# MengAiDev/SmokePhysAI

Hardware: AMD Instinct MI355X
Metric: simulated+encoded frames/sec at 256^2 grid, batch 64 (higher is better)
Workload: dtype f32 stencil + bf16x3 encoder (split-bf16 MFMA, fp32 accumulate)

## Files before the change

### smokephysai_amd/csrc/encoder.hip

```cpp
#include "encoder.h"

#include <stdlib.h>

#include "encoder_tile.h"

namespace smk {

typedef float f32x16 __attribute__((ext_vector_type(16)));

constexpr int ENC_TH = 8, ENC_TW = 32;
constexpr int ENC_AH = ENC_TH + 2, ENC_AW = ENC_TW + 2;
constexpr int ENC_XH = ENC_TH + 8, ENC_XW = ENC_TW + 8;
constexpr int ENC_ACS = ENC_AH * ENC_AW;

__global__ void k_fold_weights(smk_encoder_weights w, EncoderDev e) {
    int t = blockIdx.x * blockDim.x + threadIdx.x;
    if (t < 64) {
        float s = w.bn1_w[t] / sqrtf(w.bn1_var[t] + 1e-5f);
        e.s1[t] = s;
        e.t1[t] = (w.conv1_b[t] - w.bn1_mean[t]) * s + w.bn1_b[t];
    }
    if (t < 128) {
        float s = w.bn2_w[t] / sqrtf(w.bn2_var[t] + 1e-5f);
        e.s2[t] = s;
        e.t2[t] = (w.conv2_b[t] - w.bn2_mean[t]) * s + w.bn2_b[t];
    }
    if (t < 64 * 49) e.w1[t] = w.conv1_w[t];
    if (t < 9 * 64 * 128) {
        int o = t % 128, c = (t / 128) % 64, tap = t / (128 * 64);
        e.w2t[t] = w.conv2_w[((size_t)o * 64 + c) * 9 + tap];
    }
    __bf16 *w1p = reinterpret_cast<__bf16 *>(e.w1p), *w2q = reinterpret_cast<__bf16 *>(e.w2q);
    if (t < 64 * 64) {
        int c = t / 64, k = t % 64, ki = k >> 3, kj = k & 7;
        float v = (ki < 7 && kj < 7) ? w.conv1_w[c * 49 + ki * 7 + kj] : 0.f;
        __bf16 hi = (__bf16)v;
        w1p[t] = hi;
        w1p[64 * 64 + t] = (__bf16)(v - (float)hi);
    }
    if (t < 36 * 128 * 16) {
        int cc = t % 16, o = (t / 16) % 128, ks = t / (16 * 128);
        int tap = ks >> 2, c = (ks & 3) * 16 + cc;
        float v = w.conv2_w[((size_t)o * 64 + c) * 9 + tap];
        __bf16 hi = (__bf16)v;
        w2q[((size_t)(ks * 2 + 0) * 128 + o) * 16 + cc] = hi;
        w2q[((size_t)(ks * 2 + 1) * 128 + o) * 16 + cc] = (__bf16)(v - (float)hi);
        __bf16 *w2s = reinterpret_cast<__bf16 *>(e.w2s);
        const int ks2 = tap * 2 + (c >> 5), c32 = c & 31;
        w2s[((size_t)(ks2 * 2 + 0) * 128 + o) * 32 + c32] = hi;
        w2s[((size_t)(ks2 * 2 + 1) * 128 + o) * 32 + c32] = (__bf16)(v - (float)hi);
    }
}

__global__ __launch_bounds__(256) void k_quant_w2(smk_encoder_weights w, EncoderDev e) {
    __shared__ float red[256];
    __shared__ int sh_h, sh_l;
    const int o = blockIdx.x, tid = threadIdx.x;
    if (tid == 0) { sh_h = 0; sh_l = 0; }
    float m = 0.f;
    for (int k = tid; k < 576; k += 256) m = fmaxf(m, fabsf(w.conv2_w[(size_t)o * 576 + k]));
    red[tid] = m;
    __syncthreads();
    for (int sft = 128; sft > 0; sft >>= 1) {
        if (tid < sft) red[tid] = fmaxf(red[tid], red[tid + sft]);
        __syncthreads();
    }
    const float wmax = red[0];
    const float sw = wmax > 0.f ? wmax / 32512.0f : 1.0f;
    if (tid == 0) e.sw2[o] = sw;
    int sum_h = 0, sum_l = 0;
    for (int k = tid; k < 576; k += 256) {
        const int c = k / 9, tap = k - 9 * c;
        const int q = (int)rintf(w.conv2_w[(size_t)o * 576 + k] / sw);
        const int h = (q + 128) >> 8, l = q - (h << 8);
        const int ks = tap * 2 + (c >> 5), cc = c & 31;
        e.w2i[((size_t)(ks * 2 + 0) * 128 + o) * 32 + cc] = (signed char)h;
        e.w2i[((size_t)(ks * 2 + 1) * 128 + o) * 32 + cc] = (signed char)l;
        sum_h += h; sum_l += l;
    }
    atomicAdd(&sh_h, sum_h);
    atomicAdd(&sh_l, sum_l);
    __syncthreads();
    if (tid == 0) { e.wsum[o] = 128 * sh_h; e.wsum[128 + o] = 128 * sh_l; }
}

hipError_t launch_fold_weights(const smk_encoder_weights &w, const EncoderDev &e, hipStream_t st) {
    hipLaunchKernelGGL(k_quant_w2, dim3(128), dim3(256), 0, st, w, e);
    int n = 9 * 64 * 128;
    hipLaunchKernelGGL(k_fold_weights, dim3((n + 255) / 256), dim3(256), 0, st, w, e);
    return hipGetLastError();
}

template <int NC>
__device__ __forceinline__ void conv1_pixel(const float (&patch)[49], const float *__restrict__ w1,
                                            const float *__restrict__ s1, const float *__restrict__ t1, int c0,
                                            float (&out)[NC]) {
#pragma unroll
    for (int cc = 0; cc < NC; ++cc) {
        const float *wc = w1 + (c0 + cc) * 49;
        float acc = 0.f;
#pragma unroll
        for (int t = 0; t < 49; ++t) acc = fmaf(patch[t], wc[t], acc);
        float y = fmaf(acc, s1[c0 + cc], t1[c0 + cc]);
        out[cc] = y > 0.f ? y : 0.f;
    }
}

__global__ __launch_bounds__(256) void k_conv1_only(const float *frames, int64_t fstride, int H, int W, EncoderDev e, float *act) {
    int b = blockIdx.z;
    int j = blockIdx.x * 64 + threadIdx.x, i = blockIdx.y * 4 + threadIdx.y;
    if (i >= H || j >= W) return;
    const float *x = frames + (size_t)b * fstride;
    float patch[49];
#pragma unroll
    for (int ki = 0; ki < 7; ++ki)
#pragma unroll
        for (int kj = 0; kj < 7; ++kj) {
            int ii = i + ki - 3, jj = j + kj - 3;
            patch[ki * 7 + kj] = (ii >= 0 && ii < H && jj >= 0 && jj < W) ? x[(size_t)ii * W + jj] : 0.f;
        }
#pragma unroll 1
    for (int c0 = 0; c0 < 64; c0 += 4) {
        float o[4];
        conv1_pixel<4>(patch, e.w1, e.s1, e.t1, c0, o);
#pragma unroll
        for (int cc = 0; cc < 4; ++cc) act[(((size_t)b * 64 + c0 + cc) * H + i) * W + j] = o[cc];
    }
}

hipError_t launch_conv1_only(const float *frames, int64_t fstride, int B, int H, int W, const EncoderDev &e, float *act,
                             hipStream_t st) {
    dim3 grid(cdiv(W, 64), cdiv(H, 4), B), block(64, 4);
    hipLaunchKernelGGL(k_conv1_only, grid, block, 0, st, frames, fstride, H, W, e, act);
    return hipGetLastError();
}

constexpr int POOL_THREADS = 256;

template <int V>
__global__ __launch_bounds__(POOL_THREADS) void k_encoder_pool_partials_tokens(const float *__restrict__ partials, float *__restrict__ features,
                                                                               int ncells, int lg_tr, int lg_tc, float inv) {
    typedef float vec_t __attribute__((ext_vector_type(V)));
    constexpr int PER = 128 / V;
    const int idx = blockIdx.x * POOL_THREADS + threadIdx.x, cell = idx / PER, o = (idx - cell * PER) * V;
    if (cell >= ncells) return;
    const int b = cell >> 10, pi = (cell >> 5) & 31, pj = cell & 31, tiles_x = 32 << lg_tc;
    const float *p = partials + (((size_t)b * (32 << lg_tr) + ((size_t)pi << lg_tr)) * tiles_x + (pj << lg_tc)) * 128 + o;
    vec_t sum = *reinterpret_cast<const vec_t *>(p);
    for (int tr = 0; tr < (1 << lg_tr); ++tr)
        for (int tc = (tr == 0); tc < (1 << lg_tc); ++tc) sum += *reinterpret_cast<const vec_t *>(p + ((size_t)tr * tiles_x + tc) * 128);
    *reinterpret_cast<vec_t *>(features + (size_t)cell * 128 + o) = sum * inv;
}

__global__ __launch_bounds__(POOL_THREADS) void k_encoder_pool_partials(const float *__restrict__ partials, float *__restrict__ features,
                                                                        int lg_tr, int lg_tc, float inv) {
    __shared__ float cells[32][129];
    const int tid = threadIdx.x, b = blockIdx.x >> 5, pi = blockIdx.x & 31, tiles_x = 32 << lg_tc;
    const float *row = partials + ((size_t)b * (32 << lg_tr) + ((size_t)pi << lg_tr)) * tiles_x * 128;
    for (int i = tid; i < 32 * 32; i += POOL_THREADS) {
        const int pj = i >> 5, o = (i & 31) * 4;
        const float *p = row + (size_t)(pj << lg_tc) * 128 + o;
        float4 sum = *reinterpret_cast<const float4 *>(p);
        for (int tr = 0; tr < (1 << lg_tr); ++tr)
            for (int tc = (tr == 0); tc < (1 << lg_tc); ++tc) {
                const float4 v = *reinterpret_cast<const float4 *>(p + ((size_t)tr * tiles_x + tc) * 128);
                sum.x += v.x; sum.y += v.y; sum.z += v.z; sum.w += v.w;
            }
        cells[pj][o] = sum.x * inv; cells[pj][o + 1] = sum.y * inv; cells[pj][o + 2] = sum.z * inv; cells[pj][o + 3] = sum.w * inv;
    }
    __syncthreads();
    for (int i = tid; i < 128 * 32; i += POOL_THREADS) {
        const int o = i >> 5, pj = i & 31;
        features[((size_t)b * 128 + o) * 1024 + pi * 32 + pj] = cells[pj][o];
    }
}

static hipError_t launch_pool_partials(const float *partials, float *features, int B, int H, bool tokens, hipStream_t st) {
    const int PS = H / 32, lg_tr = PS == 16 ? 1 : 2, lg_tc = lg_tr - 1;
    const float inv = 1.0f / (float)(PS * PS);
    if (!tokens) {
        hipLaunchKernelGGL(k_encoder_pool_partials, dim3(B * 32), dim3(POOL_THREADS), 0, st, partials, features, lg_tr, lg_tc, inv);
    } else if ((reinterpret_cast<uintptr_t>(features) & 15) == 0) {
        hipLaunchKernelGGL(k_encoder_pool_partials_tokens<4>, dim3(B * 1024 * 32 / POOL_THREADS), dim3(POOL_THREADS), 0, st, partials,
                           features, B * 1024, lg_tr, lg_tc, inv);
    } else {
        hipLaunchKernelGGL(k_encoder_pool_partials_tokens<1>, dim3(B * 1024 * 128 / POOL_THREADS), dim3(POOL_THREADS), 0, st, partials,
                           features, B * 1024, lg_tr, lg_tc, inv);
    }
    return hipGetLastError();
}

void EncoderPartials::release() {
    if (buf) (void)hipFree(buf);
    for (void *p : retired) (void)hipFree(p);
    retired.clear();
    buf = nullptr;
    floats = 0;
}

hipError_t EncoderPartials::acquire(int B, int H, int W, hipStream_t st, float **out) {
    *out = nullptr;
    if (H / 32 < 16) return hipSuccess;
    const size_t need = (size_t)B * (H / B3_TH) * (W / B3_TW) * 128;
    std::lock_guard<std::mutex> lk(mu);
    if (floats < need) {
        hipStreamCaptureStatus cs = hipStreamCaptureStatusNone;
        if (hipStreamIsCapturing(st, &cs) != hipSuccess) (void)hipGetLastError();
        if (cs != hipStreamCaptureStatusNone) return hipErrorStreamCaptureUnsupported;
        float *p = nullptr;
        const hipError_t err = hipMalloc((void **)&p, need * sizeof(float));
        if (err != hipSuccess) return err;
        if (buf) retired.push_back(buf);
        buf = p;
        floats = need;
    }
    *out = buf;
    return hipSuccess;
}

constexpr int LDS_XS = ENC_XH * ENC_XW;
constexpr int LDS_A1 = 64 * ENC_ACS;
constexpr int LDS_W2 = 64 * 128;
constexpr int LDS_F32_TOTAL = LDS_XS + LDS_A1 + 2 * LDS_W2;
constexpr int A2_PITCH = 129;

template <int PS>
__global__ __launch_bounds__(512) void k_encoder_f32(const float *__restrict__ frames, int64_t fstride, int H, int W,
                                                     EncoderDev e, float *__restrict__ features) {
    extern __shared__ __attribute__((aligned(16))) float lds[];
    float *xs = lds, *a1s = lds + LDS_XS, *w2s = lds + LDS_XS + LDS_A1;
    const int tid = threadIdx.x, lane = tid & 63;
    const int wave = __builtin_amdgcn_readfirstlane(tid >> 6);
    const int b = blockIdx.z, r0 = blockIdx.y * ENC_TH, c0 = blockIdx.x * ENC_TW;
    const float *x = frames + (size_t)b * fstride;

    for (int k = tid; k < LDS_XS; k += 512) {
        int ii = r0 - 4 + k / ENC_XW, jj = c0 - 4 + k % ENC_XW;
        xs[k] = (ii >= 0 && ii < H && jj >= 0 && jj < W) ? x[(size_t)ii * W + jj] : 0.f;
    }
    float4 wreg[4];
    {
        const float4 *src = reinterpret_cast<const float4 *>(e.w2t);
#pragma unroll
        for (int q = 0; q < 4; ++q) wreg[q] = src[q * 512 + tid];
    }
    __syncthreads();

    for (int task = wave; task < 48; task += 8) {
        const int chunk = task % 6, cq = task / 6;
        const int pix = chunk * 64 + lane;
        if (pix < ENC_ACS) {
            const int ar = pix / ENC_AW, ac = pix % ENC_AW;
            const int ii = r0 - 1 + ar, jj = c0 - 1 + ac;
            float o[8];
            if (ii >= 0 && ii < H && jj >= 0 && jj < W) {
                float patch[49];
#pragma unroll
                for (int ki = 0; ki < 7; ++ki)
#pragma unroll
                    for (int kj = 0; kj < 7; ++kj) patch[ki * 7 + kj] = xs[(ar + ki) * ENC_XW + ac + kj];
                conv1_pixel<8>(patch, e.w1, e.s1, e.t1, cq * 8, o);
            } else {
#pragma unroll
                for (int cc = 0; cc < 8; ++cc) o[cc] = 0.f;
            }
#pragma unroll
            for (int cc = 0; cc < 8; ++cc) a1s[(cq * 8 + cc) * ENC_ACS + pix] = o[cc];
        }
    }
    {
        float4 *dst = reinterpret_cast<float4 *>(w2s);
#pragma unroll
        for (int q = 0; q < 4; ++q) dst[q * 512 + tid] = wreg[q];
    }
    __syncthreads();

    f32x16 acc[4];
#pragma unroll
    for (int n = 0; n < 4; ++n)
#pragma unroll
        for (int r = 0; r < 16; ++r) acc[n][r] = 0.f;
    const int l31 = lane & 31, hi = lane >> 5;
    for (int tap = 0; tap < 9; ++tap) {
        if (tap + 1 < 9) {
            const float4 *src = reinterpret_cast<const float4 *>(e.w2t + (size_t)(tap + 1) * LDS_W2);
#pragma unroll
            for (int q = 0; q < 4; ++q) wreg[q] = src[q * 512 + tid];
        }
        const int ki = tap / 3, kj = tap % 3;
        const float *ap = a1s + hi * ENC_ACS + (wave + ki) * ENC_AW + l31 + kj;
        const float *bp = w2s + (tap & 1) * LDS_W2 + hi * 128 + l31;
#pragma unroll 4
        for (int cp = 0; cp < 32; ++cp) {
            float a = ap[cp * 2 * ENC_ACS];
#pragma unroll
            for (int n = 0; n < 4; ++n) {
                float bv = bp[cp * 2 * 128 + n * 32];
                acc[n] = __builtin_amdgcn_mfma_f32_32x32x2f32(a, bv, acc[n], 0, 0, 0);
            }
        }
        if (tap + 1 < 9) {
            float4 *dst = reinterpret_cast<float4 *>(w2s + ((tap + 1) & 1) * LDS_W2);
#pragma unroll
            for (int q = 0; q < 4; ++q) dst[q * 512 + tid] = wreg[q];
        }
        __syncthreads();
    }

    float *a2s = lds;
#pragma unroll
    for (int n = 0; n < 4; ++n) {
        const int o = n * 32 + l31;
        const float s = e.s2[o], t = e.t2[o];
#pragma unroll
        for (int r = 0; r < 16; ++r) {
            const int col = (r & 3) + 8 * (r >> 2) + 4 * hi;
            float y = fmaf(acc[n][r], s, t);
            a2s[(wave * ENC_TW + col) * A2_PITCH + o] = y > 0.f ? y : 0.f;
        }
    }
    __syncthreads();
    if constexpr (PS >= 16) {
        if (tid < 256) {
            const int o = tid & 127, half = tid >> 7;
            float sum = 0.f;
            for (int rr = 0; rr < ENC_TH; ++rr)
                for (int q = 0; q < B3_TW; ++q) sum += a2s[(rr * ENC_TW + half * B3_TW + q) * A2_PITCH + o];
            const size_t tile = ((size_t)b * (H / B3_TH) + blockIdx.y) * (W / B3_TW) + 2 * blockIdx.x + half;
            features[tile * 128 + o] = sum;
        }
    } else {
        constexpr int CELLS_R = ENC_TH / PS, CELLS_C = ENC_TW / PS;
        const int OW = 32, OHW = 32 * 32;
        for (int k = tid; k < CELLS_R * CELLS_C * 128; k += 512) {
            const int o = k & 127, cell = k >> 7, cr = cell / CELLS_C, cc = cell % CELLS_C;
            float sum = 0.f;
            for (int rr = 0; rr < PS; ++rr)
                for (int q = 0; q < PS; ++q) sum += a2s[((cr * PS + rr) * ENC_TW + cc * PS + q) * A2_PITCH + o];
            const int pi = r0 / PS + cr, pj = c0 / PS + cc;
            features[((size_t)b * 128 + o) * OHW + pi * OW + pj] = sum * (1.0f / (PS * PS));
        }
    }
}

hipError_t launch_encoder_f32(const float *frames, int64_t fstride, int B, int H, int W, const EncoderDev &e,
                              float *features, hipStream_t st, float *partials) {
    const int PS = H / 32;
    if (PS >= 16 && !partials) return hipErrorInvalidValue;
    dim3 grid(W / ENC_TW, H / ENC_TH, B), block(512);
    size_t lds_bytes = sizeof(float) * (size_t)(LDS_F32_TOTAL > 256 * A2_PITCH ? LDS_F32_TOTAL : 256 * A2_PITCH);
    once_per_device((const void *)k_encoder_f32<8>, [&] {
        (void)hipFuncSetAttribute((const void *)k_encoder_f32<2>, hipFuncAttributeMaxDynamicSharedMemorySize, (int)lds_bytes);
        (void)hipFuncSetAttribute((const void *)k_encoder_f32<4>, hipFuncAttributeMaxDynamicSharedMemorySize, (int)lds_bytes);
        (void)hipFuncSetAttribute((const void *)k_encoder_f32<8>, hipFuncAttributeMaxDynamicSharedMemorySize, (int)lds_bytes);
        (void)hipFuncSetAttribute((const void *)k_encoder_f32<16>, hipFuncAttributeMaxDynamicSharedMemorySize, (int)lds_bytes);
    });
    switch (PS) {
        case 2: hipLaunchKernelGGL(k_encoder_f32<2>, grid, block, lds_bytes, st, frames, fstride, H, W, e, features); break;
        case 4: hipLaunchKernelGGL(k_encoder_f32<4>, grid, block, lds_bytes, st, frames, fstride, H, W, e, features); break;
        case 8: hipLaunchKernelGGL(k_encoder_f32<8>, grid, block, lds_bytes, st, frames, fstride, H, W, e, features); break;
        case 16:
        case 32: {
            hipLaunchKernelGGL(k_encoder_f32<16>, grid, block, lds_bytes, st, frames, fstride, H, W, e, partials);
            const hipError_t err = hipGetLastError();
            return err != hipSuccess ? err : launch_pool_partials(partials, features, B, H, false, st);
        }
        default: return hipErrorInvalidValue;
    }
    return hipGetLastError();
}

typedef __bf16 bf16x4 __attribute__((ext_vector_type(4)));

constexpr int B3_XH = B3_TH + 9, B3_XW = B3_TW + 9;
constexpr int B3_XS_BYTES = ((B3_XH * B3_XW * 4 + 15) / 16) * 16;
constexpr int B3_A1_PITCH = 144;
constexpr int B3_A1_ROW = B3_AW * B3_A1_PITCH + 32;
constexpr int B3_A1_BYTES = (B3_TH + 2) * B3_A1_ROW;
template <bool X3> constexpr int b3_lds_bytes() { return B3_XS_BYTES + (X3 ? 2 : 1) * B3_A1_BYTES; }

template <bool X3>
__device__ __forceinline__ void mma3(f32x16 &acc, const bf16x8 &ah, const bf16x8 &al, const bf16x8 &bh, const bf16x8 &bl) {
    if (X3) {
        acc = __builtin_amdgcn_mfma_f32_32x32x16_bf16(al, bh, acc, 0, 0, 0);
        acc = __builtin_amdgcn_mfma_f32_32x32x16_bf16(ah, bl, acc, 0, 0, 0);
    }
    acc = __builtin_amdgcn_mfma_f32_32x32x16_bf16(ah, bh, acc, 0, 0, 0);
}

__device__ __forceinline__ float bn_relu(float a, float s, float t) {
    float y = fmaf(a, s, t);
    return y > 0.f ? y : 0.f;
}

constexpr int B3_W1_PITCH = 144;
constexpr int B3_W1_BYTES = 64 * B3_W1_PITCH;
constexpr int B3_ST_BYTES = 2 * 64 * 4;
template <bool X3> constexpr int b3_lds_total() { return b3_lds_bytes<X3>() + (X3 ? 2 : 1) * B3_W1_BYTES + B3_ST_BYTES; }

struct SkipArgs {
    const unsigned long long *masks = nullptr;
    int *count = nullptr;
    const float *table = nullptr;
    int nbands = 0, lg_band_tiles = 0, bands_per_frame = 0;
};
constexpr int scan_rows_for(int tiles_x) { return tiles_x <= 16 ? 4 : 64 / tiles_x; }
constexpr int ENC_FRAME_FEATS = 128 * 1024;
constexpr int SKIP_CHUNKS = 256, SKIP_SLATE = 16;
struct SkipLds {
    int cpre[SKIP_CHUNKS + 1];
    int wsum[4];
    int slate[SKIP_SLATE];
};

__device__ __forceinline__ int skip_lookup(const SkipLds &s, const SkipArgs &sa, int k) {
    int c = 0;
#pragma unroll
    for (int step = SKIP_CHUNKS / 2; step >= 1; step >>= 1)
        if (s.cpre[c + step] <= k) c += step;
    int n = k - s.cpre[c];
    int j = c * ((sa.nbands + SKIP_CHUNKS - 1) / SKIP_CHUNKS);
    unsigned long long m = sa.masks[j];
    for (int pc = __popcll(m); n >= pc; pc = __popcll(m)) {
        n -= pc;
        m = sa.masks[++j];
    }
    int pos = 0;
#pragma unroll
    for (int w = 32; w >= 1; w >>= 1) {
        const int cnt = __popcll((m >> pos) & ((1ull << w) - 1));
        if (n >= cnt) {
            n -= cnt;
            pos += w;
        }
    }
    return (j << sa.lg_band_tiles) + pos;
}

__device__ __forceinline__ void skip_slate(SkipLds &s, const SkipArgs &sa, int r0, int nrun) {
    const int i = threadIdx.x;
    if (i < SKIP_SLATE) {
        const long long k = (long long)blockIdx.x + (long long)(r0 + i) * gridDim.x;
        if (k < nrun) s.slate[i] = skip_lookup(s, sa, (int)k);
    }
}

__device__ __forceinline__ int tiles_to_run(SkipLds &s, const SkipArgs &sa, int ntiles) {
    if (!sa.masks) return ntiles;
    const int tid = threadIdx.x, lane = tid & 63, wave = tid >> 6;
    const int cs = (sa.nbands + SKIP_CHUNKS - 1) / SKIP_CHUNKS;
    int c = 0;
    for (int j = tid * cs, je = min(j + cs, sa.nbands); j < je; ++j) c += __popcll(sa.masks[j]);
    int inc = c;
#pragma unroll
    for (int d = 1; d < 64; d <<= 1) {
        const int v = __shfl_up(inc, d);
        if (lane >= d) inc += v;
    }
    if (lane == 63) s.wsum[wave] = inc;
    __syncthreads();
    int base = 0;
    for (int w = 0; w < wave; ++w) base += s.wsum[w];
    s.cpre[tid] = base + inc - c;
    if (tid == SKIP_CHUNKS - 1) s.cpre[SKIP_CHUNKS] = base + inc;
    __syncthreads();
    const int nrun = __builtin_amdgcn_readfirstlane(s.cpre[SKIP_CHUNKS]);
    if (blockIdx.x == 0 && tid == 0) *sa.count = nrun;
    if (nrun != ntiles) {
        skip_slate(s, sa, 0, nrun);
        __syncthreads();
    }
    return nrun;
}
__device__ __forceinline__ int tile_at(SkipLds &s, const SkipArgs &sa, bool listed, int round, int k, int nrun) {
    if (!listed) return k;
    if (round > 0 && (round & (SKIP_SLATE - 1)) == 0) {
        skip_slate(s, sa, round, nrun);
        __syncthreads();
    }
    return __builtin_amdgcn_readfirstlane(s.slate[round & (SKIP_SLATE - 1)]);
}

template <int PS, bool TOKENS>
__device__ __forceinline__ void skip_fill(const SkipArgs &sa, int lg_tiles_x, float *__restrict__ features) {
    constexpr bool PART = PS >= 16;
    constexpr int CR = PART ? 1 : B3_TH / PS, CC = PART ? 1 : B3_TW / PS;
    constexpr int VW = TOKENS || PART ? 4 : (CC < 4 ? CC : 4), VPR = TOKENS || PART ? 1 : CC / VW, ROWV = CC * 32;
    constexpr int UPT = TOKENS || PART ? CR * ROWV : 128 * CR * VPR;
    constexpr int UNR = 4;
    typedef float vec_t __attribute__((ext_vector_type(VW)));
    const int tid = threadIdx.x, tiles_x = 1 << lg_tiles_x, band_tiles = 1 << sa.lg_band_tiles, total = band_tiles * UPT;
    const unsigned long long full = band_tiles == 64 ? ~0ull : (1ull << band_tiles) - 1;
    for (int band = blockIdx.x; band < sa.nbands; band += gridDim.x) {
        const unsigned long long mv = sa.masks[band];
        const unsigned long long m = ((unsigned long long)__builtin_amdgcn_readfirstlane((unsigned int)(mv >> 32)) << 32) |
                                     (unsigned int)__builtin_amdgcn_readfirstlane((unsigned int)mv);
        if (m == full) continue;
        const int lg_rows = PART ? sa.lg_band_tiles - lg_tiles_x : 2;
        const int b = band / sa.bands_per_frame, ty0 = (band - b * sa.bands_per_frame) << lg_rows;
        float *out = features + (size_t)b * (PART ? (size_t)sa.bands_per_frame << (sa.lg_band_tiles + 7) : (size_t)ENC_FRAME_FEATS);
        for (int i0 = tid; i0 < total; i0 += 256 * UNR) {
            vec_t v[UNR];
            int off[UNR];
#pragma unroll
            for (int j = 0; j < UNR; ++j) {
                const int i = i0 + 256 * j, tl = i / UPT, u = i - tl * UPT;
                off[j] = -1;
                if (i >= total || ((m >> tl) & 1)) continue;
                const int ty = ty0 + (tl >> lg_tiles_x), tx = tl & (tiles_x - 1);
                if (PART) {
                    off[j] = ((ty << lg_tiles_x) + tx) * 128 + u * 4;
                } else if (TOKENS) {
                    const int a = u / ROWV, q = u - a * ROWV;
                    off[j] = ((ty * CR + a) * 32 + tx * CC) * 128 + q * 4;
                } else {
                    const int vv = u % VPR, a = (u / VPR) % CR, o = u / (VPR * CR);
                    off[j] = o * 1024 + (ty * CR + a) * 32 + tx * CC + vv * VW;
                }
                v[j] = *reinterpret_cast<const vec_t *>(sa.table + off[j]);
            }
#pragma unroll
            for (int j = 0; j < UNR; ++j)
                if (off[j] >= 0) __builtin_nontemporal_store(v[j], reinterpret_cast<vec_t *>(out + off[j]));
        }
    }
}
__device__ __forceinline__ bool skip_fill_first() { return (blockIdx.x / 256) & 1; }


template <int PARTS>
__device__ __forceinline__ void conv1_stage(const EncoderDev &e, unsigned char *w1s, float *st1) {
    const int tid = threadIdx.x;
    if (tid < 128) st1[tid] = tid < 64 ? e.s1[tid] : e.t1[tid - 64];
    const uint4 *src = reinterpret_cast<const uint4 *>(e.w1p);
    for (int c = tid; c < PARTS * 64 * 8; c += 256) {
        const int row = c >> 3, u = c & 7;
        *reinterpret_cast<uint4 *>(w1s + row * B3_W1_PITCH + u * 16) = src[c];
    }
}

struct TileSrc {
    const float *frames;
    int64_t fstride;
    int H, W, lg_tiles_x, lg_tiles_per_frame;
    __device__ __forceinline__ void decode(int t, int &b, int &r0, int &c0) const {
        b = t >> lg_tiles_per_frame;
        const int rem = t & ((1 << lg_tiles_per_frame) - 1);
        r0 = (rem >> lg_tiles_x) * B3_TH;
        c0 = (rem & ((1 << lg_tiles_x) - 1)) * B3_TW;
    }
    __device__ __forceinline__ float fetch(int t, int k) const {
        if (k >= B3_XH * B3_XW) return 0.f;
        int bb, rr0, cc0;
        decode(t, bb, rr0, cc0);
        const int row = k / B3_XW, col = k - row * B3_XW;
        const int ii = rr0 - 4 + row, jj = cc0 - 4 + col;
        const bool ok = row < B3_XH - 1 && col < B3_XW - 1 && ii >= 0 && ii < H && jj >= 0 && jj < W;
        return ok ? frames[(size_t)bb * fstride + (size_t)ii * W + jj] : 0.f;
    }
};

template <class T, class Word>
__device__ __forceinline__ void halo_to_lds(T *xs, float v0, float v1, Word word) {
    const int tid = threadIdx.x;
    xs[tid] = word(v0);
    if (tid + 256 < B3_XH * B3_XW) xs[tid + 256] = word(v1);
}

struct TileWalk {
    int k, nrun, round, t, tn;
    bool listed;

    template <int PS, bool TOKENS, class T, class Word>
    __device__ __forceinline__ void begin(SkipLds &skl, const SkipArgs &sa, const TileSrc &src, int ntiles, int stagger,
                                          float *__restrict__ features, T *xs, Word word) {
        k = blockIdx.x;
        nrun = tiles_to_run(skl, sa, ntiles);
        listed = nrun != ntiles;
        round = 0;
        t = k < nrun ? tile_at(skl, sa, listed, 0, k, nrun) : 0;
        if (listed && skip_fill_first()) skip_fill<PS, TOKENS>(sa, src.lg_tiles_x, features);
        else if (stagger > 0 && ((blockIdx.x / 256) & 1))
            for (int i = 0; i < stagger; ++i) __builtin_amdgcn_s_sleep(127);
        const int tid = threadIdx.x;
        if (k < nrun) halo_to_lds(xs, src.fetch(t, tid), src.fetch(t, tid + 256), word);
        __syncthreads();
    }
    __device__ __forceinline__ void next(SkipLds &skl, const SkipArgs &sa, const TileSrc &src, float &xr0, float &xr1) {
        const int kn = k + gridDim.x;
        ++round;
        tn = kn < nrun ? tile_at(skl, sa, listed, round, kn, nrun) : 0;
        xr0 = 0.f;
        xr1 = 0.f;
        if (kn < nrun) {
            const int tid = threadIdx.x;
            xr0 = src.fetch(tn, tid);
            xr1 = src.fetch(tn, tid + 256);
        }
    }
    template <int PS, bool TOKENS>
    __device__ __forceinline__ void end(const SkipArgs &sa, const TileSrc &src, float *__restrict__ features) const {
        if (listed && !skip_fill_first()) {
            __builtin_amdgcn_s_setprio(0);
            skip_fill<PS, TOKENS>(sa, src.lg_tiles_x, features);
        }
    }
};

template <int A1_ROW, int A1_PITCH>
__device__ __forceinline__ void x_frags(const float *xs, int pb, int r0, int c0, int H, int W, bf16x8 (&xh)[4], bf16x8 (&xl)[4],
                                        int &aoff, bool &valid, bool &inimg) {
    const int r = threadIdx.x & 31, hi = (threadIdx.x >> 5) & 1;
    const int pix = pb * 32 + r;
    valid = pix < B3_APIX;
    const int pc = valid ? pix : B3_APIX - 1;
    const int ar = pc / B3_AW, ac = pc - ar * B3_AW;
    const int ii = r0 - 1 + ar, jj = c0 - 1 + ac;
    inimg = valid && ii >= 0 && ii < H && jj >= 0 && jj < W;
    aoff = ar * A1_ROW + ac * A1_PITCH;
    const float *xp = xs + (ar + hi) * B3_XW + ac;
#pragma unroll
    for (int s = 0; s < 4; ++s)
#pragma unroll
        for (int j = 0; j < 8; ++j) {
            __bf16 vh, vl;
            split_bf16(xp[s * 2 * B3_XW + j], vh, vl);
            xh[s][j] = vh; xl[s][j] = vl;
        }
}

template <bool X3>
__device__ __forceinline__ void conv1_both(const unsigned char *w1s, const bf16x8 (&xh)[4], const bf16x8 (&xl)[4], f32x16 &acc0,
                                           f32x16 &acc1) {
    const int r = threadIdx.x & 31, hi = (threadIdx.x >> 5) & 1;
#pragma unroll
    for (int g = 0; g < 16; ++g) { acc0[g] = 0.f; acc1[g] = 0.f; }
    const unsigned char *wrow = w1s + r * B3_W1_PITCH + 8 * hi * 2;
#pragma unroll
    for (int s = 0; s < 4; ++s) {
        const bf16x8 a0h = *reinterpret_cast<const bf16x8 *>(wrow + s * 32);
        const bf16x8 a1hh = *reinterpret_cast<const bf16x8 *>(wrow + 32 * B3_W1_PITCH + s * 32);
        const bf16x8 a0l = X3 ? *reinterpret_cast<const bf16x8 *>(wrow + B3_W1_BYTES + s * 32) : a0h;
        const bf16x8 a1l_ = X3 ? *reinterpret_cast<const bf16x8 *>(wrow + B3_W1_BYTES + 32 * B3_W1_PITCH + s * 32) : a1hh;
        mma3<X3>(acc0, a0h, a0l, xh[s], xl[s]);
        mma3<X3>(acc1, a1hh, a1l_, xh[s], xl[s]);
    }
}
template <bool X3>
__device__ __forceinline__ void conv1_one(const unsigned char *w1s, int cb, const bf16x8 (&xh)[4], const bf16x8 (&xl)[4],
                                          f32x16 &acc) {
    const int r = threadIdx.x & 31, hi = (threadIdx.x >> 5) & 1;
#pragma unroll
    for (int g = 0; g < 16; ++g) acc[g] = 0.f;
    const unsigned char *wrow = w1s + (cb * 32 + r) * B3_W1_PITCH + 8 * hi * 2;
#pragma unroll
    for (int s = 0; s < 4; ++s) {
        const bf16x8 ah = *reinterpret_cast<const bf16x8 *>(wrow + s * 32);
        const bf16x8 al = X3 ? *reinterpret_cast<const bf16x8 *>(wrow + B3_W1_BYTES + s * 32) : ah;
        mma3<X3>(acc, ah, al, xh[s], xl[s]);
    }
}

template <int PS, bool TOKENS, class Val>
__device__ __forceinline__ void pool_store_32(float *__restrict__ features, int b, int o, int r0, int c0, int tile, Val val) {
    const int hi = (threadIdx.x >> 5) & 1;
    auto out_index = [&](int pi, int pj) -> size_t {
        return TOKENS ? ((size_t)b * 1024 + pi * 32 + pj) * 128 + o : ((size_t)b * 128 + o) * 1024 + pi * 32 + pj;
    };
    if (PS == 2) {
#pragma unroll
        for (int mp = 0; mp < 2; ++mp)
#pragma unroll
            for (int qr = 0; qr < 2; ++qr)
#pragma unroll
                for (int qc = 0; qc < 2; ++qc)
#pragma unroll
                    for (int cg = 0; cg < 2; ++cg) {
                        float sum = 0.f;
#pragma unroll
                        for (int mi = 2 * mp; mi < 2 * mp + 2; ++mi)
#pragma unroll
                            for (int i = 2 * cg; i < 2 * cg + 2; ++i) sum += val(mi, 4 * (2 * qr + qc) + i);
                        features[out_index((r0 + 2 * mp + 4 * qr) / 2, (c0 + 8 * qc + 4 * hi + 2 * cg) / 2)] = sum * 0.25f;
                    }
    } else if (PS == 4) {
#pragma unroll
        for (int qr = 0; qr < 2; ++qr)
#pragma unroll
            for (int qc = 0; qc < 2; ++qc) {
                float sum = 0.f;
#pragma unroll
                for (int mi = 0; mi < 4; ++mi)
#pragma unroll
                    for (int i = 0; i < 4; ++i) sum += val(mi, 4 * (2 * qr + qc) + i);
                features[out_index((r0 + 4 * qr) / 4, (c0 + 8 * qc + 4 * hi) / 4)] = sum * (1.0f / 16);
            }
    } else if (PS >= 16) {
        float cell[2];
#pragma unroll
        for (int qc = 0; qc < 2; ++qc) {
            float sum = 0.f;
#pragma unroll
            for (int mi = 0; mi < 4; ++mi)
#pragma unroll
                for (int qr = 0; qr < 2; ++qr)
#pragma unroll
                    for (int i = 0; i < 4; ++i) sum += val(mi, 4 * (2 * qr + qc) + i);
            cell[qc] = sum;
        }
        const float mine = cell[0] + cell[1];
        const float total = mine + __shfl_xor(mine, 32);
        if (hi == 0) features[(size_t)tile * 128 + o] = total;
    } else {
        float cell[2];
#pragma unroll
        for (int qc = 0; qc < 2; ++qc) {
            float sum = 0.f;
#pragma unroll
            for (int mi = 0; mi < 4; ++mi)
#pragma unroll
                for (int qr = 0; qr < 2; ++qr)
#pragma unroll
                    for (int i = 0; i < 4; ++i) sum += val(mi, 4 * (2 * qr + qc) + i);
            cell[qc] = sum;
        }
        const float other0 = __shfl_xor(cell[0], 32), other1 = __shfl_xor(cell[1], 32);
        const float total = hi == 0 ? cell[0] + other0 : cell[1] + other1;
        features[out_index(r0 / 8, c0 / 8 + hi)] = total * (1.0f / 64);
    }
}

template <bool X3, int PS, bool TOKENS>
__global__ __launch_bounds__(256, 2) void k_encoder_bf16(const float *__restrict__ frames, int64_t fstride, int H, int W,
                                                      EncoderDev e, float *__restrict__ features, int lg_tiles_x,
                                                      int lg_tiles_per_frame, int ntiles, int stagger,
                                                      SkipArgs sa) {
    extern __shared__ __attribute__((aligned(16))) unsigned char smem[];
    float *xs = reinterpret_cast<float *>(smem);
    unsigned char *a1h = smem + B3_XS_BYTES, *a1l = a1h + B3_A1_BYTES;
    unsigned char *w1s = a1h + (X3 ? 2 : 1) * B3_A1_BYTES;
    float *st1 = reinterpret_cast<float *>(w1s + (X3 ? 2 : 1) * B3_W1_BYTES);
    const int tid = threadIdx.x, lane = tid & 63, r = lane & 31, hi = lane >> 5;
    const int wave = __builtin_amdgcn_readfirstlane(tid >> 6);

    conv1_stage<X3 ? 2 : 1>(e, w1s, st1);
    const int o = wave * 32 + r;
    const float s2 = e.s2[o], t2 = e.t2[o];
    const int lane_b = (o * 2 + hi) * 16;
    const __amdgpu_buffer_rsrc_t wrsrc =
        __builtin_amdgcn_make_buffer_rsrc(const_cast<unsigned short *>(e.w2q), 0, 36 * 2 * 4096, 0x00020000);
    typedef unsigned int u32x4 __attribute__((ext_vector_type(4)));
    auto load_b = [&](int kn, int part) -> uint4 {
        const u32x4 v = __builtin_amdgcn_raw_buffer_load_b128(wrsrc, lane_b, (kn * 2 + part) * 4096, 0);
        return make_uint4(v[0], v[1], v[2], v[3]);
    };
    constexpr int RING = 6;
    uint4 bqh[RING], bql[RING];
#pragma unroll
    for (int k = 0; k < RING - 1; ++k) {
        bqh[k] = load_b(k, 0);
        if (X3) bql[k] = load_b(k, 1);
    }
    const int lane_off = (r >> 4) * 4 * B3_A1_ROW + (r & 15) * B3_A1_PITCH + 8 * hi * 2;

    const TileSrc src{frames, fstride, H, W, lg_tiles_x, lg_tiles_per_frame};
    __shared__ SkipLds skl;
    TileWalk wk;
    wk.begin<PS, TOKENS>(skl, sa, src, ntiles, stagger, features, xs, [](float v) { return v; });

    for (; wk.k < wk.nrun; wk.k += gridDim.x) {
        int b, r0, c0;
        src.decode(wk.t, b, r0, c0);

        __builtin_amdgcn_s_setprio(0);
        auto conv1_store = [&](const f32x16 &acc, int cb, int aoff, bool valid, bool inimg) {
#pragma unroll
            for (int q = 0; q < 4; ++q) {
                const int ch0 = cb * 32 + 8 * q + 4 * hi;
                const float4 sc = *reinterpret_cast<const float4 *>(st1 + ch0);
                const float4 sh = *reinterpret_cast<const float4 *>(st1 + 64 + ch0);
                const float scv[4] = {sc.x, sc.y, sc.z, sc.w}, shv[4] = {sh.x, sh.y, sh.z, sh.w};
                bf16x4 vh, vl;
#pragma unroll
                for (int i = 0; i < 4; ++i) {
                    const float y = inimg ? bn_relu(acc[4 * q + i], scv[i], shv[i]) : 0.f;
                    __bf16 a, bb;
                    split_bf16(y, a, bb);
                    vh[i] = a; vl[i] = bb;
                }
                if (valid) {
                    *reinterpret_cast<bf16x4 *>(a1h + aoff + ch0 * 2) = vh;
                    if (X3) *reinterpret_cast<bf16x4 *>(a1l + aoff + ch0 * 2) = vl;
                }
            }
        };
        {
            bf16x8 xh[4], xl[4];
            int aoff; bool valid, inimg;
            x_frags<B3_A1_ROW, B3_A1_PITCH>(xs, wave, r0, c0, H, W, xh, xl, aoff, valid, inimg);
            f32x16 acc0, acc1;
            conv1_both<X3>(w1s, xh, xl, acc0, acc1);
            conv1_store(acc0, 0, aoff, valid, inimg);
            conv1_store(acc1, 1, aoff, valid, inimg);
        }
        {
            bf16x8 xh[4], xl[4];
            int aoff; bool valid, inimg;
            const int cb = wave & 1;
            x_frags<B3_A1_ROW, B3_A1_PITCH>(xs, 4 + (wave >> 1), r0, c0, H, W, xh, xl, aoff, valid, inimg);
            f32x16 acc;
            conv1_one<X3>(w1s, cb, xh, xl, acc);
            conv1_store(acc, cb, aoff, valid, inimg);
        }
        __syncthreads();
        __builtin_amdgcn_s_setprio(1);

        float xr0, xr1;
        wk.next(skl, sa, src, xr0, xr1);

        f32x16 acc[4];
#pragma unroll
        for (int mi = 0; mi < 4; ++mi)
#pragma unroll
            for (int g = 0; g < 16; ++g) acc[mi][g] = 0.f;
        auto load_a = [&](int k, bf16x8 (&ah)[4], bf16x8 (&al)[4]) {
            const int tap = k >> 2, ks = k & 3, ki = tap / 3, kj = tap - 3 * ki;
            const int abase = lane_off + ki * B3_A1_ROW + kj * B3_A1_PITCH + ks * 32;
#pragma unroll
            for (int mi = 0; mi < 4; ++mi) {
                ah[mi] = *reinterpret_cast<const bf16x8 *>(a1h + abase + mi * B3_A1_ROW);
                if (X3) al[mi] = *reinterpret_cast<const bf16x8 *>(a1l + abase + mi * B3_A1_ROW);
            }
        };
        bf16x8 ahA[4], alA[4], ahB[4], alB[4];
        load_a(0, ahA, alA);
        constexpr int UNR = 6;
#pragma unroll 1
        for (int k0 = 0; k0 < 36; k0 += UNR) {
#pragma unroll
            for (int u = 0; u < UNR; ++u) {
                const int k = k0 + u;
                {
                    int kn = k + RING - 1;
                    kn = kn >= 36 ? kn - 36 : kn;
                    kn = __builtin_amdgcn_readfirstlane(kn);
                    bqh[(u + RING - 1) % RING] = load_b(kn, 0);
                    if (X3) bql[(u + RING - 1) % RING] = load_b(kn, 1);
                }
                if (k + 1 < 36) {
                    if (u & 1) load_a(k + 1, ahA, alA); else load_a(k + 1, ahB, alB);
                }
                const bf16x8 bh = __builtin_bit_cast(bf16x8, bqh[u % RING]);
                const bf16x8 bl = X3 ? __builtin_bit_cast(bf16x8, bql[u % RING]) : bh;
#pragma unroll
                for (int mi = 0; mi < 4; ++mi) {
                    if (u & 1) mma3<X3>(acc[mi], ahB[mi], alB[mi], bh, bl); else mma3<X3>(acc[mi], ahA[mi], alA[mi], bh, bl);
                }
                constexpr int NMF = X3 ? 12 : 4, NDS = X3 ? 8 : 4, NVM = X3 ? 2 : 1;
#pragma unroll
                for (int i = 0; i < NMF; ++i) {
                    __builtin_amdgcn_sched_group_barrier(0x008, 1, 0);
                    if (i < NDS) __builtin_amdgcn_sched_group_barrier(0x100, 1, 0);
                    else if (i < NDS + NVM) __builtin_amdgcn_sched_group_barrier(0x020, 1, 0);
                }
                __builtin_amdgcn_sched_barrier(0);
            }
        }

        pool_store_32<PS, TOKENS>(features, b, o, r0, c0, wk.t, [&](int mi, int g) { return bn_relu(acc[mi][g], s2, t2); });

        halo_to_lds(xs, xr0, xr1, [](float v) { return v; });
        __syncthreads();
        wk.t = wk.tn;
    }
    wk.end<PS, TOKENS>(sa, src, features);
}

constexpr int S16_LDS = B3_XS_BYTES + 2 * S16_A1_BYTES + 2 * B3_W1_BYTES + B3_ST_BYTES;

template <int PS, bool TOKENS>
__global__ __launch_bounds__(256, 2) void k_encoder_b16(const float *__restrict__ frames, int64_t fstride, int H, int W,
                                                     EncoderDev e, float *__restrict__ features, int lg_tiles_x,
                                                     int lg_tiles_per_frame, int ntiles, int stagger,
                                                     SkipArgs sa) {
    extern __shared__ __attribute__((aligned(16))) unsigned char smem[];
    unsigned int *xs = reinterpret_cast<unsigned int *>(smem);
    unsigned char *a1h = smem + B3_XS_BYTES, *a1l = a1h + S16_A1_BYTES;
    unsigned char *w1s = a1l + S16_A1_BYTES;
    float *st1 = reinterpret_cast<float *>(w1s + 2 * B3_W1_BYTES);
    const int tid = threadIdx.x, lane = tid & 63, r = lane & 31, hi = lane >> 5;
    const int wave = __builtin_amdgcn_readfirstlane(tid >> 6);

    conv1_stage<2>(e, w1s, st1);
    const int px = lane & 15, kg = lane >> 4;
    const int o0 = wave * 32 + px;
    const float s2a = e.s2[o0], t2a = e.t2[o0], s2b = e.s2[o0 + 16], t2b = e.t2[o0 + 16];
    const int lane_b = o0 * 64 + kg * 16;
    const __amdgpu_buffer_rsrc_t wrsrc =
        __builtin_amdgcn_make_buffer_rsrc(const_cast<unsigned short *>(e.w2s), 0, 18 * 2 * 8192, 0x00020000);
    typedef unsigned int u32x4 __attribute__((ext_vector_type(4)));
    auto load_b = [&](int ks, int part, int nt) -> uint4 {
        const u32x4 v = __builtin_amdgcn_raw_buffer_load_b128(wrsrc, lane_b, (ks * 2 + part) * 8192 + nt * 1024, 0);
        return make_uint4(v.x, v.y, v.z, v.w);
    };
    constexpr int RING = 2;
    uint4 bq[RING][2][2];
#pragma unroll
    for (int k = 0; k < RING - 1; ++k)
#pragma unroll
        for (int nt = 0; nt < 2; ++nt) {
            bq[k][nt][0] = load_b(k, 0, nt);
            bq[k][nt][1] = load_b(k, 1, nt);
        }

    auto pack_split = [](float v) -> unsigned int {
        __bf16 vh, vl;
        split_bf16(v, vh, vl);
        return (unsigned int)__builtin_bit_cast(unsigned short, vh) | ((unsigned int)__builtin_bit_cast(unsigned short, vl) << 16);
    };
    const TileSrc src{frames, fstride, H, W, lg_tiles_x, lg_tiles_per_frame};
    __shared__ SkipLds skl;
    TileWalk wk;
    wk.begin<PS, TOKENS>(skl, sa, src, ntiles, stagger, features, xs, pack_split);

    for (; wk.k < wk.nrun; wk.k += gridDim.x) {
        int b, r0, c0;
        src.decode(wk.t, b, r0, c0);

        __builtin_amdgcn_s_setprio(S16_PRIO_CONV1);
#ifdef SMK_ENC_ABLATE
        const bool abl_conv1 = !((SMK_ENC_ABLATE & 1) && wk.k != (int)blockIdx.x);
#else
        constexpr bool abl_conv1 = true;
#endif
        auto x_frags = [&](int pb, bf16x8 (&xh)[4], bf16x8 (&xl)[4], int &pix, bool &valid, bool &inimg) {
            const int pp = pb * 32 + r;
            valid = pp < B3_APIX;
            pix = valid ? pp : B3_APIX - 1;
            const int ar = pix / B3_AW, ac = pix - ar * B3_AW;
            const int ii = r0 - 1 + ar, jj = c0 - 1 + ac;
            inimg = valid && ii >= 0 && ii < H && jj >= 0 && jj < W;
            const unsigned int *xp = xs + (ar + hi) * B3_XW + ac;
#pragma unroll
            for (int s = 0; s < 4; ++s) {
                unsigned int wh[4], wl[4];
#pragma unroll
                for (int jj = 0; jj < 4; ++jj) {
                    const unsigned int e0 = xp[s * 2 * B3_XW + 2 * jj], e1 = xp[s * 2 * B3_XW + 2 * jj + 1];
                    wh[jj] = __builtin_amdgcn_perm(e1, e0, 0x05040100u);
                    wl[jj] = __builtin_amdgcn_perm(e1, e0, 0x07060302u);
                }
                xh[s] = __builtin_bit_cast(bf16x8, make_uint4(wh[0], wh[1], wh[2], wh[3]));
                xl[s] = __builtin_bit_cast(bf16x8, make_uint4(wl[0], wl[1], wl[2], wl[3]));
            }
        };
        auto conv1_store = [&](const f32x16 &acc, int cb, int pix, bool valid, bool inimg) {
            const int sw = pix & 7;
#pragma unroll
            for (int q = 0; q < 4; ++q) {
                const int ch0 = cb * 32 + 8 * q + 4 * hi;
                const float4 sc = *reinterpret_cast<const float4 *>(st1 + ch0);
                const float4 sh = *reinterpret_cast<const float4 *>(st1 + 64 + ch0);
                const float scv[4] = {sc.x, sc.y, sc.z, sc.w}, shv[4] = {sh.x, sh.y, sh.z, sh.w};
                bf16x4 vh, vl;
#pragma unroll
                for (int i = 0; i < 4; ++i) {
                    const float y = inimg ? bn_relu(acc[4 * q + i], scv[i], shv[i]) : 0.f;
                    __bf16 a, bb;
                    split_bf16(y, a, bb);
                    vh[i] = a; vl[i] = bb;
                }
                if (valid) {
                    const int off = pix * 128 + (((cb * 4 + q) ^ sw) * 16) + 8 * hi;
                    *reinterpret_cast<bf16x4 *>(a1h + off) = vh;
                    *reinterpret_cast<bf16x4 *>(a1l + off) = vl;
                }
            }
        };
        if (abl_conv1) {
            bf16x8 xh[4], xl[4];
            int pix; bool valid, inimg;
            x_frags(wave, xh, xl, pix, valid, inimg);
            f32x16 acc0, acc1;
            conv1_both<true>(w1s, xh, xl, acc0, acc1);
            conv1_store(acc0, 0, pix, valid, inimg);
            conv1_store(acc1, 1, pix, valid, inimg);
        }
        if (abl_conv1) {
            bf16x8 xh[4], xl[4];
            int pix; bool valid, inimg;
            const int cb = wave & 1;
            x_frags(4 + (wave >> 1), xh, xl, pix, valid, inimg);
            f32x16 acc;
            conv1_one<true>(w1s, cb, xh, xl, acc);
            conv1_store(acc, cb, pix, valid, inimg);
        }
#if !defined(SMK_ENC_ABLATE) || !(SMK_ENC_ABLATE & 4)
        __syncthreads();
#endif
        __builtin_amdgcn_s_setprio(S16_PRIO_KLOOP);

        float xr0, xr1;
        wk.next(skl, sa, src, xr0, xr1);

        f32x4v acc[8][2];
#pragma unroll
        for (int mt = 0; mt < 8; ++mt)
#pragma unroll
            for (int nt = 0; nt < 2; ++nt)
#pragma unroll
                for (int g = 0; g < 4; ++g) acc[mt][nt][g] = 0.f;
        const int c16[2] = {kg << 4, (4 + kg) << 4};
        auto tap_consts = [&](int ki, int kj, int (&om)[4]) {
#pragma unroll
            for (int m = 0; m < 4; ++m) om[m] = ((px + kj) << 7) ^ (((px + kj + 2 * (m + ki)) & 7) << 4);
        };
        auto load_a = [&](int ki, int half, int hm, const int (&om)[4], bf16x8 (&ah)[4], bf16x8 (&al)[4]) {
            const unsigned char *ph = a1h + ki * (B3_AW * 128), *pl = a1l + ki * (B3_AW * 128);
#pragma unroll
            for (int m = 0; m < 4; ++m) {
                const int off = om[m] ^ c16[half];
                ah[m] = *reinterpret_cast<const bf16x8 *>(ph + off + (4 * hm + m) * (B3_AW * 128));
                al[m] = *reinterpret_cast<const bf16x8 *>(pl + off + (4 * hm + m) * (B3_AW * 128));
            }
        };
        bf16x8 ahA[4], alA[4], ahB[4], alB[4];
        int om[4];
        tap_consts(0, 0, om);
        load_a(0, 0, 0, om, ahA, alA);
        int ki = 0, kj = 0;
#pragma unroll 1
        for (int tap = 0; tap < 9; ++tap) {
#pragma unroll
            for (int u = 0; u < 4; ++u) {
                const int half = u >> 1, hm = u & 1, slot = half % RING;
                if (hm == 0) {
                    int kn = tap * 2 + half + RING - 1;
                    kn = kn >= 18 ? kn - 18 : kn;
                    kn = __builtin_amdgcn_readfirstlane(kn);
#pragma unroll
                    for (int nt = 0; nt < 2; ++nt) {
                        bq[(slot + RING - 1) % RING][nt][0] = load_b(kn, 0, nt);
                        bq[(slot + RING - 1) % RING][nt][1] = load_b(kn, 1, nt);
                    }
                }
                if (u < 3) {
                    if (u & 1) load_a(ki, (u + 1) >> 1, (u + 1) & 1, om, ahA, alA);
                    else load_a(ki, (u + 1) >> 1, (u + 1) & 1, om, ahB, alB);
                } else if (tap < 8) {
                    kj = kj == 2 ? 0 : kj + 1;
                    ki = kj == 0 ? ki + 1 : ki;
                    tap_consts(ki, kj, om);
                    load_a(ki, 0, 0, om, ahA, alA);
                }
#pragma unroll
                for (int pr = 0; pr < 3; ++pr)
#pragma unroll
                    for (int m = 0; m < 4; ++m)
#pragma unroll
                        for (int nt = 0; nt < 2; ++nt) {
                            const bf16x8 bh = __builtin_bit_cast(bf16x8, bq[slot][nt][0]);
                            const bf16x8 bl = __builtin_bit_cast(bf16x8, bq[slot][nt][1]);
                            f32x4v &c = acc[4 * hm + m][nt];
                            const bf16x8 ah = (u & 1) ? ahB[m] : ahA[m], al = (u & 1) ? alB[m] : alA[m];
#if defined(SMK_ENC_ABLATE) && (SMK_ENC_ABLATE & 8)
                            asm volatile("" :: "v"(al), "v"(ah), "v"(bh), "v"(bl), "v"(c));
#else
                            if (pr == 0) c = __builtin_amdgcn_mfma_f32_16x16x32_bf16(al, bh, c, 0, 0, 0);
                            else if (pr == 1) c = __builtin_amdgcn_mfma_f32_16x16x32_bf16(ah, bl, c, 0, 0, 0);
                            else c = __builtin_amdgcn_mfma_f32_16x16x32_bf16(ah, bh, c, 0, 0, 0);
#endif
                        }
#pragma unroll
                for (int i = 0; i < 24; ++i) {
                    __builtin_amdgcn_sched_group_barrier(0x008, 1, 0);
                    if (i % 3 == 0) __builtin_amdgcn_sched_group_barrier(0x100, 1, 0);
                    else if (hm == 0 && (i == 1 || i == 2 || i == 4 || i == 5)) __builtin_amdgcn_sched_group_barrier(0x020, 1, 0);
                }
                __builtin_amdgcn_sched_barrier(0);
            }
        }

        auto out_index = [&](int pi, int pj, int o) -> size_t {
            return TOKENS ? ((size_t)b * 1024 + pi * 32 + pj) * 128 + o : ((size_t)b * 128 + o) * 1024 + pi * 32 + pj;
        };
#if defined(SMK_ENC_ABLATE) && (SMK_ENC_ABLATE & 2)
#pragma unroll
        for (int mt = 0; mt < 8; ++mt) asm volatile("" :: "v"(acc[mt][0]), "v"(acc[mt][1]));
        if (false)
#endif
#pragma unroll
        for (int nt = 0; nt < 2; ++nt) {
            const float s2 = nt ? s2b : s2a, t2 = nt ? t2b : t2a;
            const int o = o0 + 16 * nt;
            if (PS == 2) {
#pragma unroll
                for (int mp = 0; mp < 4; ++mp)
#pragma unroll
                    for (int cg = 0; cg < 2; ++cg) {
                        float sum = 0.f;
#pragma unroll
                        for (int mt = 2 * mp; mt < 2 * mp + 2; ++mt)
#pragma unroll
                            for (int i = 2 * cg; i < 2 * cg + 2; ++i) sum += bn_relu(acc[mt][nt][i], s2, t2);
                        features[out_index((r0 + 2 * mp) / 2, (c0 + 4 * kg + 2 * cg) / 2, o)] = sum * 0.25f;
                    }
            } else if (PS == 4) {
#pragma unroll
                for (int mq = 0; mq < 2; ++mq) {
                    float sum = 0.f;
#pragma unroll
                    for (int mt = 4 * mq; mt < 4 * mq + 4; ++mt)
#pragma unroll
                        for (int i = 0; i < 4; ++i) sum += bn_relu(acc[mt][nt][i], s2, t2);
                    features[out_index((r0 + 4 * mq) / 4, (c0 + 4 * kg) / 4, o)] = sum * (1.0f / 16);
                }
            } else if (PS >= 16) {
                float sum = 0.f;
#pragma unroll
                for (int mt = 0; mt < 8; ++mt)
#pragma unroll
                    for (int i = 0; i < 4; ++i) sum += bn_relu(acc[mt][nt][i], s2, t2);
                const float half8 = sum + __shfl_xor(sum, 16);
                const float total = half8 + __shfl_xor(half8, 32);
                if (kg == 0) features[(size_t)wk.t * 128 + o] = total;
            } else {
                float sum = 0.f;
#pragma unroll
                for (int mt = 0; mt < 8; ++mt)
#pragma unroll
                    for (int i = 0; i < 4; ++i) sum += bn_relu(acc[mt][nt][i], s2, t2);
                const float other = __shfl_xor(sum, 16);
                const float total = (kg & 1) == 0 ? sum + other : other + sum;
                if ((kg & 1) == 0) features[out_index(r0 / 8, c0 / 8 + (kg >> 1), o)] = total * (1.0f / 64);
            }
        }

        halo_to_lds(xs, xr0, xr1, pack_split);
#if !defined(SMK_ENC_ABLATE) || !(SMK_ENC_ABLATE & 4)
        __syncthreads();
#endif
        wk.t = wk.tn;
    }
    wk.end<PS, TOKENS>(sa, src, features);
}

struct EncoderKnobs {
    int stagger, wgs_per_cu, shape;
    bool skip;
    EncoderKnobs() {
        const char *sv = getenv("SMK_ENC_STAGGER"), *ov = getenv("SMK_ENC_WGS_PER_CU"), *sh = getenv("SMK_ENC_SHAPE");
        const char *sk = getenv("SMK_ENC_SKIP");
        stagger = sv ? atoi(sv) : 1;
        wgs_per_cu = ov && atoi(ov) > 0 ? atoi(ov) : 0;
        shape = sh && atoi(sh) == 32 ? 32 : 16;
        skip = !(sk && atoi(sk) == 0);
    }
};
static const EncoderKnobs &enc_knobs() {
    static const EncoderKnobs k;
    return k;
}

template <bool VEC, int ROWS>
__global__ __launch_bounds__(256) void k_encoder_tile_scan(const float *__restrict__ frames, int64_t fstride, int H, int W, int lg_tiles_x,
                                                           int bands_per_frame, unsigned long long *__restrict__ masks) {
    constexpr int SCAN_ROWS = ROWS;
    constexpr int SCAN_BR = 2 * ROWS + 2;
    constexpr int SCAN_FW = 1024 / ROWS / 4 + 2;
    __shared__ unsigned int flag[SCAN_BR][SCAN_FW];
    const int tid = threadIdx.x;
    const int band = blockIdx.x, b = band / bands_per_frame, bi = band - b * bands_per_frame;
    const int tiles_x = 1 << lg_tiles_x, band_tiles = SCAN_ROWS * tiles_x;
    for (int i = tid; i < SCAN_BR * SCAN_FW; i += 256) (&flag[0][0])[i] = 0;
    __syncthreads();
    const int W4 = W >> 2, row0 = bi * (SCAN_ROWS * B3_TH) - 4;
    const unsigned int *src = reinterpret_cast<const unsigned int *>(frames) + (size_t)b * fstride;
    for (int i = tid; i < SCAN_BR * 4 * W4; i += 256) {
        const int rr = i / W4, c4 = i - rr * W4, row = row0 + rr;
        if (row < 0 || row >= H) continue;
        const unsigned int *p = src + (size_t)row * W + 4 * c4;
        unsigned int any;
        if (VEC) {
            const uint4 v = *reinterpret_cast<const uint4 *>(p);
            any = v.x | v.y | v.z | v.w;
        } else {
            any = p[0] | p[1] | p[2] | p[3];
        }
        if (any) flag[rr >> 2][c4 + 1] = 1;
    }
    __syncthreads();
    if (tid < 64) {
        unsigned int any = 0;
        if (tid < band_tiles) {
            const int tyl = tid >> lg_tiles_x, tx = tid & (tiles_x - 1);
#pragma unroll
            for (int br = 0; br < 4; ++br)
#pragma unroll
                for (int bc = 0; bc < 6; ++bc) any |= flag[2 * tyl + br][4 * tx + bc];
        }
        const unsigned long long m = __ballot(any != 0);
        if (tid == 0) masks[band] = m;
    }
}

void EncoderSkip::release() {
    for (auto &f : table)
        for (auto &h : f)
            for (float *&t : h) {
                if (t) (void)hipFree(t);
                t = nullptr;
            }
    if (ws) (void)hipFree(ws);
    for (void *p : retired) (void)hipFree(p);
    retired.clear();
    ws = nullptr;
    ws_bands = 0;
    last_count = nullptr;
}

hipError_t encoder_skip_stats(EncoderSkip &sk, int64_t *tiles_total, int64_t *tiles_run, hipStream_t st) {
    std::lock_guard<std::mutex> lk(sk.mu);
    hipError_t err = hipStreamSynchronize(st);
    if (err != hipSuccess) return err;
    int n = 0;
    if (sk.last_count && (err = hipMemcpy(&n, sk.last_count, sizeof(int), hipMemcpyDeviceToHost)) != hipSuccess) return err;
    *tiles_total = sk.last_total;
    *tiles_run = sk.last_count ? n : sk.last_total;
    return hipSuccess;
}

template <int FORM, bool TOKENS, class ZeroLaunch>
static hipError_t skip_prepare(EncoderSkip *sk, const float *frames, int64_t fstride, int B, int H, int W, float *features, int lg_tx,
                               int ntiles, int nwg, hipStream_t st, ZeroLaunch zero_launch, SkipArgs &plan) {
    if (!sk) return hipSuccess;
    std::lock_guard<std::mutex> lk(sk->mu);
    sk->last_total = ntiles;
    sk->last_count = nullptr;
    if (!enc_knobs().skip || ntiles <= nwg || (reinterpret_cast<uintptr_t>(features) & 15)) return hipSuccess;
    hipStreamCaptureStatus cs = hipStreamCaptureStatusNone;
    if (hipStreamIsCapturing(st, &cs) != hipSuccess) {
        (void)hipGetLastError();
        return hipSuccess;
    }
    const bool capturing = cs != hipStreamCaptureStatusNone;
    hipError_t err;
    const bool part = H / 32 >= 16;
    const int hidx = H == 64 ? 0 : H == 128 ? 1 : H == 256 ? 2 : H == 512 ? 3 : 4;
    if (H != 64 && H != 128 && H != 256 && H != 512 && H != 1024) return hipErrorInvalidValue;
    float *&tab = sk->table[FORM][hidx][TOKENS && !part ? 1 : 0];
    if (!tab) {
        if (capturing) return hipSuccess;
        const size_t tfloats = part ? (size_t)(H / B3_TH) * (W / B3_TW) * 128 : (size_t)ENC_FRAME_FEATS;
        float *p = nullptr;
        if ((err = hipMalloc((void **)&p, (tfloats + (size_t)H * W) * sizeof(float))) != hipSuccess) return err;
        err = hipMemsetAsync(p + tfloats, 0, (size_t)H * W * sizeof(float), st);
        if (err == hipSuccess) err = zero_launch(p + tfloats, p);
        if (err != hipSuccess) {
            (void)hipFree(p);
            return err;
        }
        tab = p;
    }
    const int scan_rows = scan_rows_for(1 << lg_tx);
    const int bands_per_frame = H / B3_TH / scan_rows, nbands = B * bands_per_frame;
    if (sk->ws_bands < (size_t)nbands) {
        if (capturing) return hipSuccess;
        int *p = nullptr;
        if ((err = hipMalloc((void **)&p, (4 + 2 * (size_t)nbands) * sizeof(int))) != hipSuccess) return err;
        if (sk->ws) sk->retired.push_back(sk->ws);
        sk->ws = p;
        sk->ws_bands = nbands;
    }
    int *count = sk->ws;
    unsigned long long *masks = reinterpret_cast<unsigned long long *>(sk->ws + 4);
    const bool vec = (reinterpret_cast<uintptr_t>(frames) & 15) == 0 && (fstride & 3) == 0;
    dim3 grid(nbands), block(256);
    auto scan = [&](auto kern) { hipLaunchKernelGGL(kern, grid, block, 0, st, frames, fstride, H, W, lg_tx, bands_per_frame, masks); };
    switch (scan_rows) {
        case 4: vec ? scan(k_encoder_tile_scan<true, 4>) : scan(k_encoder_tile_scan<false, 4>); break;
        case 2: vec ? scan(k_encoder_tile_scan<true, 2>) : scan(k_encoder_tile_scan<false, 2>); break;
        default: vec ? scan(k_encoder_tile_scan<true, 1>) : scan(k_encoder_tile_scan<false, 1>); break;
    }
    if ((err = hipGetLastError()) != hipSuccess) return err;
    plan.masks = masks;
    plan.count = count;
    plan.nbands = nbands;
    plan.lg_band_tiles = lg_tx + 2 < 6 ? lg_tx + 2 : 6;
    plan.table = tab;
    plan.bands_per_frame = bands_per_frame;
    sk->last_count = count;
    return hipSuccess;
}

typedef int i32x16 __attribute__((ext_vector_type(16)));
typedef int i32x4 __attribute__((ext_vector_type(4)));

constexpr int I8_A1_PITCH = 80;
constexpr int I8_A1_ROW = B3_AW * I8_A1_PITCH + 32;
constexpr int I8_A1_BYTES = (B3_TH + 2) * I8_A1_ROW;
constexpr int I8_LDS_BYTES = B3_XS_BYTES + 2 * I8_A1_BYTES + 2 * B3_W1_BYTES + B3_ST_BYTES + 64;

template <int PS, bool TOKENS>
__global__ __launch_bounds__(256, 2) void k_encoder_i8(const float *__restrict__ frames, int64_t fstride, int H, int W,
                                                    EncoderDev e, float *__restrict__ features, int lg_tiles_x,
                                                    int lg_tiles_per_frame, int ntiles,
                                                    SkipArgs sa) {
    extern __shared__ __attribute__((aligned(16))) unsigned char smem[];
    float *xs = reinterpret_cast<float *>(smem);
    unsigned char *a1h = smem + B3_XS_BYTES, *a1l = a1h + I8_A1_BYTES;
    unsigned char *w1s = a1l + I8_A1_BYTES;
    float *st1 = reinterpret_cast<float *>(w1s + 2 * B3_W1_BYTES);
    float *wmx = st1 + 128;
    const int tid = threadIdx.x, lane = tid & 63, r = lane & 31, hi = lane >> 5;
    const int wave = __builtin_amdgcn_readfirstlane(tid >> 6);

    conv1_stage<2>(e, w1s, st1);
    const int o = wave * 32 + r;
    const float t2 = e.t2[o];
    const float scale_o = e.sw2[o] * e.s2[o];
    const int corr_h = e.wsum[o], corr_l = e.wsum[128 + o];
    const int lane_b = (o * 2 + hi) * 16;
    const __amdgpu_buffer_rsrc_t wrsrc =
        __builtin_amdgcn_make_buffer_rsrc(const_cast<signed char *>(e.w2i), 0, 18 * 2 * 4096, 0x00020000);
    typedef unsigned int u32x4 __attribute__((ext_vector_type(4)));
    auto load_b = [&](int kn, int part) -> i32x4 {
        const u32x4 v = __builtin_amdgcn_raw_buffer_load_b128(wrsrc, lane_b, (kn * 2 + part) * 4096, 0);
        return __builtin_bit_cast(i32x4, v);
    };
    constexpr int RING = 3;
    i32x4 bqh[RING], bql[RING];
#pragma unroll
    for (int k = 0; k < RING - 1; ++k) {
        bqh[k] = load_b(k, 0);
        bql[k] = load_b(k, 1);
    }
    const int lane_off = (r >> 4) * 4 * I8_A1_ROW + (r & 15) * I8_A1_PITCH + 16 * hi;

    const TileSrc src{frames, fstride, H, W, lg_tiles_x, lg_tiles_per_frame};
    __shared__ SkipLds skl;
    TileWalk wk;
    wk.begin<PS, TOKENS>(skl, sa, src, ntiles, 0, features, xs, [](float v) { return v; });

    for (; wk.k < wk.nrun; wk.k += gridDim.x) {
        int b, r0, c0;
        src.decode(wk.t, b, r0, c0);

        __builtin_amdgcn_s_setprio(0);
        float yv[3][16];
        int aoffs[2];
        bool valids[2];
        float vmax = 0.f;
        bool inimgs[2];
        auto bn1 = [&](const f32x16 &acc, int cb, bool inimg, float (&y)[16]) {
            float umax = 0.f;
#pragma unroll
            for (int q = 0; q < 4; ++q) {
                const int ch0 = cb * 32 + 8 * q + 4 * hi;
                const float4 sc = *reinterpret_cast<const float4 *>(st1 + ch0);
                const float4 sh = *reinterpret_cast<const float4 *>(st1 + 64 + ch0);
                const float scv[4] = {sc.x, sc.y, sc.z, sc.w}, shv[4] = {sh.x, sh.y, sh.z, sh.w};
#pragma unroll
                for (int i = 0; i < 4; ++i) {
                    const float v = bn_relu(acc[4 * q + i], scv[i], shv[i]);
                    y[4 * q + i] = v;
                    umax = fmaxf(umax, v);
                }
            }
            vmax = fmaxf(vmax, inimg ? umax : 0.f);
        };
        {
            bf16x8 xh[4], xl[4];
            bool inimg;
            x_frags<I8_A1_ROW, I8_A1_PITCH>(xs, wave, r0, c0, H, W, xh, xl, aoffs[0], valids[0], inimg);
            inimgs[0] = inimg;
            f32x16 acc0, acc1;
            conv1_both<true>(w1s, xh, xl, acc0, acc1);
            bn1(acc0, 0, inimg, yv[0]);
            bn1(acc1, 1, inimg, yv[1]);
        }
        const int cbs = wave & 1;
        {
            bf16x8 xh[4], xl[4];
            bool inimg;
            x_frags<I8_A1_ROW, I8_A1_PITCH>(xs, 4 + (wave >> 1), r0, c0, H, W, xh, xl, aoffs[1], valids[1], inimg);
            inimgs[1] = inimg;
            f32x16 acc;
            conv1_one<true>(w1s, cbs, xh, xl, acc);
            bn1(acc, cbs, inimg, yv[2]);
        }
#pragma unroll
        for (int off = 32; off > 0; off >>= 1) vmax = fmaxf(vmax, __shfl_xor(vmax, off));
        if (lane == 0) wmx[wave] = vmax;
        __syncthreads();
        const float tmax = fmaxf(fmaxf(wmx[0], wmx[1]), fmaxf(wmx[2], wmx[3]));
        const float invn = tmax > 0.f ? 65024.0f / (tmax * 65535.0f) : 0.f;
        const float s_tile = tmax > 0.f ? tmax / 65024.0f : 0.f;
        constexpr float OFFN = 128.0f / 65535.0f;
        auto quant_store = [&](const float (&y)[16], int cb, int aoff, bool valid, bool inimg) {
            if (!valid) return;
#pragma unroll
            for (int q = 0; q < 4; ++q) {
                const int ch0 = cb * 32 + 8 * q + 4 * hi;
                const unsigned int d0 = __builtin_bit_cast(unsigned int, __builtin_amdgcn_cvt_pknorm_u16(
                    fmaf(y[4 * q + 0], invn, OFFN), fmaf(y[4 * q + 1], invn, OFFN)));
                const unsigned int d1 = __builtin_bit_cast(unsigned int, __builtin_amdgcn_cvt_pknorm_u16(
                    fmaf(y[4 * q + 2], invn, OFFN), fmaf(y[4 * q + 3], invn, OFFN)));
                unsigned int ph = __builtin_amdgcn_perm(d1, d0, 0x07050301) ^ 0x80808080u;
                unsigned int pl = __builtin_amdgcn_perm(d1, d0, 0x06040200) ^ 0x80808080u;
                ph = inimg ? ph : 0x80808080u;
                pl = inimg ? pl : 0u;
                *reinterpret_cast<unsigned int *>(a1h + aoff + ch0) = ph;
                *reinterpret_cast<unsigned int *>(a1l + aoff + ch0) = pl;
            }
        };
        quant_store(yv[0], 0, aoffs[0], valids[0], inimgs[0]);
        quant_store(yv[1], 1, aoffs[0], valids[0], inimgs[0]);
        quant_store(yv[2], cbs, aoffs[1], valids[1], inimgs[1]);
        __syncthreads();
        __builtin_amdgcn_s_setprio(1);

        float xr0, xr1;
        wk.next(skl, sa, src, xr0, xr1);

        i32x16 hh[4], mid[4];
#pragma unroll
        for (int mi = 0; mi < 4; ++mi)
#pragma unroll
            for (int g = 0; g < 16; ++g) { hh[mi][g] = corr_h; mid[mi][g] = corr_l; }
        auto load_a = [&](int k, int pair, i32x4 (&ah)[2], i32x4 (&al)[2]) {
            const int tap = k >> 1, half = k & 1, ki = tap / 3, kj = tap - 3 * ki;
            const int abase = lane_off + ki * I8_A1_ROW + kj * I8_A1_PITCH + half * 32 + pair * 2 * I8_A1_ROW;
#pragma unroll
            for (int m = 0; m < 2; ++m) {
                ah[m] = *reinterpret_cast<const i32x4 *>(a1h + abase + m * I8_A1_ROW);
                al[m] = *reinterpret_cast<const i32x4 *>(a1l + abase + m * I8_A1_ROW);
            }
        };
        i32x4 ahA[2], alA[2], ahB[2], alB[2];
        load_a(0, 0, ahA, alA);
#pragma unroll 1
        for (int k0 = 0; k0 < 18; k0 += 6) {
#pragma unroll
            for (int u = 0; u < 6; ++u) {
                const int k = k0 + u;
                {
                    int kn = k + RING - 1;
                    kn = kn >= 18 ? kn - 18 : kn;
                    kn = __builtin_amdgcn_readfirstlane(kn);
                    bqh[(u + RING - 1) % RING] = load_b(kn, 0);
                    bql[(u + RING - 1) % RING] = load_b(kn, 1);
                }
                const i32x4 bh = bqh[u % RING], bl = bql[u % RING];
                load_a(k, 1, ahB, alB);
#pragma unroll
                for (int m = 0; m < 2; ++m) {
                    mid[m] = __builtin_amdgcn_mfma_i32_32x32x32_i8(alA[m], bh, mid[m], 0, 0, 0);
                    mid[m] = __builtin_amdgcn_mfma_i32_32x32x32_i8(ahA[m], bl, mid[m], 0, 0, 0);
                    hh[m] = __builtin_amdgcn_mfma_i32_32x32x32_i8(ahA[m], bh, hh[m], 0, 0, 0);
                }
#pragma unroll
                for (int i = 0; i < 6; ++i) {
                    __builtin_amdgcn_sched_group_barrier(0x008, 1, 0);
                    if (i < 4) __builtin_amdgcn_sched_group_barrier(0x100, 1, 0);
                    else __builtin_amdgcn_sched_group_barrier(0x020, 1, 0);
                }
                __builtin_amdgcn_sched_barrier(0);
                if (k + 1 < 18) load_a(k + 1, 0, ahA, alA);
#pragma unroll
                for (int m = 0; m < 2; ++m) {
                    mid[2 + m] = __builtin_amdgcn_mfma_i32_32x32x32_i8(alB[m], bh, mid[2 + m], 0, 0, 0);
                    mid[2 + m] = __builtin_amdgcn_mfma_i32_32x32x32_i8(ahB[m], bl, mid[2 + m], 0, 0, 0);
                    hh[2 + m] = __builtin_amdgcn_mfma_i32_32x32x32_i8(ahB[m], bh, hh[2 + m], 0, 0, 0);
                }
#pragma unroll
                for (int i = 0; i < 6; ++i) {
                    __builtin_amdgcn_sched_group_barrier(0x008, 1, 0);
                    if (i < 4) __builtin_amdgcn_sched_group_barrier(0x100, 1, 0);
                }
                __builtin_amdgcn_sched_barrier(0);
            }
        }

        const float sc = s_tile * scale_o * 256.0f;
        auto val = [&](int mi, int g) -> float {
            const float v = fmaf((float)hh[mi][g], 256.0f, (float)mid[mi][g]);
            const float y = fmaf(v, sc, t2);
            return y > 0.f ? y : 0.f;
        };
        pool_store_32<PS, TOKENS>(features, b, o, r0, c0, wk.t, val);

        halo_to_lds(xs, xr0, xr1, [](float v) { return v; });
        __syncthreads();
        wk.t = wk.tn;
    }
    wk.end<PS, TOKENS>(sa, src, features);
}

struct FormB16 {
    static constexpr int FORM = 0, LDS = S16_LDS;
    static constexpr bool STAGGERS = true;
    template <int PS, bool TOKENS> static constexpr auto kernel = &k_encoder_b16<PS, TOKENS>;
};
template <bool X3>
struct FormBf16 {
    static constexpr int FORM = X3 ? 0 : 1, LDS = b3_lds_total<X3>();
    static constexpr bool STAGGERS = true;
    template <int PS, bool TOKENS> static constexpr auto kernel = &k_encoder_bf16<X3, PS, TOKENS>;
};
struct FormI8 {
    static constexpr int FORM = 2, LDS = I8_LDS_BYTES;
    static constexpr bool STAGGERS = false;
    template <int PS, bool TOKENS> static constexpr auto kernel = &k_encoder_i8<PS, TOKENS>;
};

template <class F, bool TOKENS>
static hipError_t launch_persistent(const float *frames, int64_t fstride, int B, int H, int W, const EncoderDev &e, float *features,
                                    hipStream_t st, EncoderSkip *skip, float *partials) {
    const int PS = H / 32;
    const int tiles_x = W / B3_TW, tiles_per_frame = tiles_x * (H / B3_TH), ntiles = B * tiles_per_frame;
    int lg_tx = 0, lg_tpf = 0;
    while ((1 << lg_tx) < tiles_x) ++lg_tx;
    while ((1 << lg_tpf) < tiles_per_frame) ++lg_tpf;
    if ((1 << lg_tx) != tiles_x || (1 << lg_tpf) != tiles_per_frame || (PS != 2 && PS != 4 && PS != 8 && PS != 16 && PS != 32))
        return hipErrorInvalidValue;
    const bool part = PS >= 16;
    if (part && !partials) return hipErrorInvalidValue;
    const int stagger = enc_knobs().stagger;
    const int num_cu = device_num_cu();
    const int wgs_per_cu = device_cached_int((const void *)F::template kernel<8, TOKENS>, [] {
        (void)hipFuncSetAttribute((const void *)F::template kernel<8, TOKENS>, hipFuncAttributeMaxDynamicSharedMemorySize, F::LDS);
        (void)hipFuncSetAttribute((const void *)F::template kernel<4, TOKENS>, hipFuncAttributeMaxDynamicSharedMemorySize, F::LDS);
        (void)hipFuncSetAttribute((const void *)F::template kernel<2, TOKENS>, hipFuncAttributeMaxDynamicSharedMemorySize, F::LDS);
        (void)hipFuncSetAttribute((const void *)F::template kernel<16, false>, hipFuncAttributeMaxDynamicSharedMemorySize, F::LDS);
        int n = 0;
        if (hipOccupancyMaxActiveBlocksPerMultiprocessor(&n, (const void *)F::template kernel<8, TOKENS>, 256, F::LDS) != hipSuccess || n < 1) n = 2;
        return enc_knobs().wgs_per_cu ? enc_knobs().wgs_per_cu : n;
    });
    auto run = [&](const float *fr, int64_t fs, int nt, float *out, const SkipArgs &sa) -> hipError_t {
        int nwg = num_cu * wgs_per_cu;
        if (nwg > nt) nwg = nt;
        dim3 grid(nwg), block(256);
        auto go = [&](auto kern) {
            if constexpr (F::STAGGERS) hipLaunchKernelGGL(kern, grid, block, F::LDS, st, fr, fs, H, W, e, out, lg_tx, lg_tpf, nt, stagger, sa);
            else hipLaunchKernelGGL(kern, grid, block, F::LDS, st, fr, fs, H, W, e, out, lg_tx, lg_tpf, nt, sa);
        };
        switch (PS) {
            case 2: go(F::template kernel<2, TOKENS>); break;
            case 4: go(F::template kernel<4, TOKENS>); break;
            case 8: go(F::template kernel<8, TOKENS>); break;
            default: go(F::template kernel<16, false>); break;
        }
        return hipGetLastError();
    };
    SkipArgs plan;
    hipError_t err = skip_prepare<F::FORM, TOKENS>(
        skip, frames, fstride, B, H, W, part ? partials : features, lg_tx, ntiles, num_cu * wgs_per_cu, st,
        [&](const float *zero_frame, float *table) { return run(zero_frame, (int64_t)H * W, tiles_per_frame, table, SkipArgs()); },
        plan);
    if (err != hipSuccess) return err;
    if (!part) return run(frames, fstride, ntiles, features, plan);
    if ((err = run(frames, fstride, ntiles, partials, plan)) != hipSuccess) return err;
    return launch_pool_partials(partials, features, B, H, TOKENS, st);
}

hipError_t launch_encoder_b16(const float *frames, int64_t fstride, int B, int H, int W, const EncoderDev &e, float *features,
                              bool tokens, hipStream_t st, EncoderSkip *skip, float *partials) {
    return tokens ? launch_persistent<FormB16, true>(frames, fstride, B, H, W, e, features, st, skip, partials)
                  : launch_persistent<FormB16, false>(frames, fstride, B, H, W, e, features, st, skip, partials);
}

hipError_t launch_encoder_bf16(const float *frames, int64_t fstride, int B, int H, int W, const EncoderDev &e,
                               float *features, bool x3, bool tokens, hipStream_t st, EncoderSkip *skip, float *partials) {
    const int shape = enc_knobs().shape;
    if (x3 && shape == 16) return launch_encoder_b16(frames, fstride, B, H, W, e, features, tokens, st, skip, partials);
    if (x3) return tokens ? launch_persistent<FormBf16<true>, true>(frames, fstride, B, H, W, e, features, st, skip, partials)
                          : launch_persistent<FormBf16<true>, false>(frames, fstride, B, H, W, e, features, st, skip, partials);
    return tokens ? launch_persistent<FormBf16<false>, true>(frames, fstride, B, H, W, e, features, st, skip, partials)
                  : launch_persistent<FormBf16<false>, false>(frames, fstride, B, H, W, e, features, st, skip, partials);
}

hipError_t launch_encoder_i8(const float *frames, int64_t fstride, int B, int H, int W, const EncoderDev &e, float *features,
                             bool tokens, hipStream_t st, EncoderSkip *skip, float *partials) {
    return tokens ? launch_persistent<FormI8, true>(frames, fstride, B, H, W, e, features, st, skip, partials)
                  : launch_persistent<FormI8, false>(frames, fstride, B, H, W, e, features, st, skip, partials);
}

}
```

Before: 237,300.

## Skip empty half-tiles in bf16 encoder by scanning left/right 8-wide cells

The tile scan now records separate activity masks for the left and right 8-column halves of each tile. For PS==8, the bf16 encoder lists tiles where only one half is active as single-cell entries and computes only that half's conv work, while skip_fill writes precomputed constant features for the inactive half. This targets wasted conv1/conv2 MFMA work on half-empty tiles in sparse smoke frames. It adds a second prefix-scan segment, extra mask traffic and branching, and is enabled by default through SMK_ENC_CELLS.

```diff
diff --git a/smokephysai_amd/csrc/encoder.hip b/smokephysai_amd/csrc/encoder.hip
--- a/smokephysai_amd/csrc/encoder.hip
+++ b/smokephysai_amd/csrc/encoder.hip
@@ -3,6 +3,7 @@
 #include <stdlib.h>
 
 #include "encoder_tile.h"
+#include "encoder_cells.h"
 
 namespace smk {
 
@@ -400,6 +401,7 @@
 
 struct SkipArgs {
     const unsigned long long *masks = nullptr;
+    const unsigned long long *cell_l = nullptr, *cell_r = nullptr;
     int *count = nullptr;
     const float *table = nullptr;
     int nbands = 0, lg_band_tiles = 0, bands_per_frame = 0;
@@ -407,23 +409,35 @@
 constexpr int scan_rows_for(int tiles_x) { return tiles_x <= 16 ? 4 : 64 / tiles_x; }
 constexpr int ENC_FRAME_FEATS = 128 * 1024;
 constexpr int SKIP_CHUNKS = 256, SKIP_SLATE = 16;
+template <bool CELLS>
 struct SkipLds {
-    int cpre[SKIP_CHUNKS + 1];
-    int wsum[4];
+    static constexpr int SEGS = CELLS ? 2 : 1;
+    int cpre[SEGS][SKIP_CHUNKS + 1];
+    int wsum[SEGS][4];
     int slate[SKIP_SLATE];
 };
-
-__device__ __forceinline__ int skip_lookup(const SkipLds &s, const SkipArgs &sa, int k) {
+template <bool CELLS>
+__device__ __forceinline__ unsigned long long skip_mask(const SkipArgs &sa, int seg, int j) {
+    if (!CELLS) return sa.masks[j];
+    const unsigned long long l = sa.cell_l[j], r = sa.cell_r[j];
+    return seg ? enc_cells_one(l, r) : enc_cells_both(l, r);
+}
+
+template <bool CELLS>
+__device__ __forceinline__ int skip_lookup(const SkipLds<CELLS> &s, const SkipArgs &sa, int k) {
+    const int seg = CELLS && k >= s.cpre[0][SKIP_CHUNKS];
+    if (seg) k -= s.cpre[0][SKIP_CHUNKS];
+    const int *cpre = s.cpre[seg];
     int c = 0;
 #pragma unroll
     for (int step = SKIP_CHUNKS / 2; step >= 1; step >>= 1)
-        if (s.cpre[c + step] <= k) c += step;
-    int n = k - s.cpre[c];
+        if (cpre[c + step] <= k) c += step;
+    int n = k - cpre[c];
     int j = c * ((sa.nbands + SKIP_CHUNKS - 1) / SKIP_CHUNKS);
-    unsigned long long m = sa.masks[j];
+    unsigned long long m = skip_mask<CELLS>(sa, seg, j);
     for (int pc = __popcll(m); n >= pc; pc = __popcll(m)) {
         n -= pc;
-        m = sa.masks[++j];
+        m = skip_mask<CELLS>(sa, seg, ++j);
     }
     int pos = 0;
 #pragma unroll
@@ -434,10 +448,13 @@
             pos += w;
         }
     }
-    return (j << sa.lg_band_tiles) + pos;
-}
-
-__device__ __forceinline__ void skip_slate(SkipLds &s, const SkipArgs &sa, int r0, int nrun) {
+    const int tile = (j << sa.lg_band_tiles) + pos;
+    if (!CELLS) return tile;
+    return enc_entry(tile, seg, (int)(~sa.cell_l[j] >> pos) & 1);
+}
+
+template <bool CELLS>
+__device__ __forceinline__ void skip_slate(SkipLds<CELLS> &s, const SkipArgs &sa, int r0, int nrun) {
     const int i = threadIdx.x;
     if (i < SKIP_SLATE) {
         const long long k = (long long)blockIdx.x + (long long)(r0 + i) * gridDim.x;
@@ -445,34 +462,46 @@
     }
 }
 
-__device__ __forceinline__ int tiles_to_run(SkipLds &s, const SkipArgs &sa, int ntiles) {
+template <bool CELLS>
+__device__ __forceinline__ int tiles_to_run(SkipLds<CELLS> &s, const SkipArgs &sa, int ntiles, bool &listed) {
+    listed = false;
     if (!sa.masks) return ntiles;
     const int tid = threadIdx.x, lane = tid & 63, wave = tid >> 6;
     const int cs = (sa.nbands + SKIP_CHUNKS - 1) / SKIP_CHUNKS;
-    int c = 0;
-    for (int j = tid * cs, je = min(j + cs, sa.nbands); j < je; ++j) c += __popcll(sa.masks[j]);
-    int inc = c;
-#pragma unroll
-    for (int d = 1; d < 64; d <<= 1) {
-        const int v = __shfl_up(inc, d);
-        if (lane >= d) inc += v;
-    }
-    if (lane == 63) s.wsum[wave] = inc;
+    int c[SkipLds<CELLS>::SEGS], inc[SkipLds<CELLS>::SEGS];
+#pragma unroll
+    for (int seg = 0; seg < SkipLds<CELLS>::SEGS; ++seg) {
+        c[seg] = 0;
+        for (int j = tid * cs, je = min(j + cs, sa.nbands); j < je; ++j) c[seg] += __popcll(skip_mask<CELLS>(sa, seg, j));
+        inc[seg] = c[seg];
+#pragma unroll
+        for (int d = 1; d < 64; d <<= 1) {
+            const int v = __shfl_up(inc[seg], d);
+            if (lane >= d) inc[seg] += v;
+        }
+        if (lane == 63) s.wsum[seg][wave] = inc[seg];
+    }
     __syncthreads();
-    int base = 0;
-    for (int w = 0; w < wave; ++w) base += s.wsum[w];
-    s.cpre[tid] = base + inc - c;
-    if (tid == SKIP_CHUNKS - 1) s.cpre[SKIP_CHUNKS] = base + inc;
+#pragma unroll
+    for (int seg = 0; seg < SkipLds<CELLS>::SEGS; ++seg) {
+        int base = 0;
+        for (int w = 0; w < wave; ++w) base += s.wsum[seg][w];
+        s.cpre[seg][tid] = base + inc[seg] - c[seg];
+        if (tid == SKIP_CHUNKS - 1) s.cpre[seg][SKIP_CHUNKS] = base + inc[seg];
+    }
     __syncthreads();
-    const int nrun = __builtin_amdgcn_readfirstlane(s.cpre[SKIP_CHUNKS]);
+    const int nfirst = __builtin_amdgcn_readfirstlane(s.cpre[0][SKIP_CHUNKS]);
+    const int nrun = CELLS ? nfirst + __builtin_amdgcn_readfirstlane(s.cpre[SkipLds<CELLS>::SEGS - 1][SKIP_CHUNKS]) : nfirst;
     if (blockIdx.x == 0 && tid == 0) *sa.count = nrun;
-    if (nrun != ntiles) {
+    listed = nfirst != ntiles;
+    if (listed) {
         skip_slate(s, sa, 0, nrun);
         __syncthreads();
     }
     return nrun;
 }
-__device__ __forceinline__ int tile_at(SkipLds &s, const SkipArgs &sa, bool listed, int round, int k, int nrun) {
+template <bool CELLS>
+__device__ __forceinline__ int tile_at(SkipLds<CELLS> &s, const SkipArgs &sa, bool listed, int round, int k, int nrun) {
     if (!listed) return k;
     if (round > 0 && (round & (SKIP_SLATE - 1)) == 0) {
         skip_slate(s, sa, round, nrun);
@@ -481,8 +510,9 @@
     return __builtin_amdgcn_readfirstlane(s.slate[round & (SKIP_SLATE - 1)]);
 }
 
-template <int PS, bool TOKENS>
+template <int PS, bool TOKENS, bool CELLS>
 __device__ __forceinline__ void skip_fill(const SkipArgs &sa, int lg_tiles_x, float *__restrict__ features) {
+    static_assert(!CELLS || PS == 8, "cells are the two halves of a tile at PS == 8 only");
     constexpr bool PART = PS >= 16;
     constexpr int CR = PART ? 1 : B3_TH / PS, CC = PART ? 1 : B3_TW / PS;
     constexpr int VW = TOKENS || PART ? 4 : (CC < 4 ? CC : 4), VPR = TOKENS || PART ? 1 : CC / VW, ROWV = CC * 32;
@@ -491,37 +521,48 @@
     typedef float vec_t __attribute__((ext_vector_type(VW)));
     const int tid = threadIdx.x, tiles_x = 1 << lg_tiles_x, band_tiles = 1 << sa.lg_band_tiles, total = band_tiles * UPT;
     const unsigned long long full = band_tiles == 64 ? ~0ull : (1ull << band_tiles) - 1;
+    auto uniform = [](unsigned long long mv) -> unsigned long long {
+        return ((unsigned long long)__builtin_amdgcn_readfirstlane((unsigned int)(mv >> 32)) << 32) |
+               (unsigned int)__builtin_amdgcn_readfirstlane((unsigned int)mv);
+    };
     for (int band = blockIdx.x; band < sa.nbands; band += gridDim.x) {
-        const unsigned long long mv = sa.masks[band];
-        const unsigned long long m = ((unsigned long long)__builtin_amdgcn_readfirstlane((unsigned int)(mv >> 32)) << 32) |
-                                     (unsigned int)__builtin_amdgcn_readfirstlane((unsigned int)mv);
+        const unsigned long long ml = uniform(CELLS ? sa.cell_l[band] : sa.masks[band]), mr = CELLS ? uniform(sa.cell_r[band]) : ml;
+        const unsigned long long m = ml & mr;
         if (m == full) continue;
         const int lg_rows = PART ? sa.lg_band_tiles - lg_tiles_x : 2;
         const int b = band / sa.bands_per_frame, ty0 = (band - b * sa.bands_per_frame) << lg_rows;
         float *out = features + (size_t)b * (PART ? (size_t)sa.bands_per_frame << (sa.lg_band_tiles + 7) : (size_t)ENC_FRAME_FEATS);
         for (int i0 = tid; i0 < total; i0 += 256 * UNR) {
             vec_t v[UNR];
-            int off[UNR];
+            int off[UNR], word[UNR];
 #pragma unroll
             for (int j = 0; j < UNR; ++j) {
                 const int i = i0 + 256 * j, tl = i / UPT, u = i - tl * UPT;
                 off[j] = -1;
+                word[j] = -1;
                 if (i >= total || ((m >> tl) & 1)) continue;
                 const int ty = ty0 + (tl >> lg_tiles_x), tx = tl & (tiles_x - 1);
+                const bool lrun = CELLS && ((ml >> tl) & 1), rrun = CELLS && ((mr >> tl) & 1);
                 if (PART) {
                     off[j] = ((ty << lg_tiles_x) + tx) * 128 + u * 4;
                 } else if (TOKENS) {
                     const int a = u / ROWV, q = u - a * ROWV;
+                    if (CELLS && (q >= 32 ? rrun : lrun)) continue;
                     off[j] = ((ty * CR + a) * 32 + tx * CC) * 128 + q * 4;
                 } else {
                     const int vv = u % VPR, a = (u / VPR) % CR, o = u / (VPR * CR);
                     off[j] = o * 1024 + (ty * CR + a) * 32 + tx * CC + vv * VW;
+                    if (CELLS && (lrun || rrun)) word[j] = lrun ? 1 : 0;
                 }
                 v[j] = *reinterpret_cast<const vec_t *>(sa.table + off[j]);
             }
 #pragma unroll
-            for (int j = 0; j < UNR; ++j)
-                if (off[j] >= 0) __builtin_nontemporal_store(v[j], reinterpret_cast<vec_t *>(out + off[j]));
+            for (int j = 0; j < UNR; ++j) {
+                if (off[j] < 0) continue;
+                if (CELLS && !TOKENS && word[j] >= 0)
+                    __builtin_nontemporal_store(word[j] ? v[j][VW - 1] : v[j][0], out + off[j] + word[j]);
+                else __builtin_nontemporal_store(v[j], reinterpret_cast<vec_t *>(out + off[j]));
+            }
         }
     }
 }
@@ -567,33 +608,41 @@
     if (tid + 256 < B3_XH * B3_XW) xs[tid + 256] = word(v1);
 }
 
+template <bool CELLS = false>
 struct TileWalk {
-    int k, nrun, round, t, tn;
+    int k, nrun, round, t, tn, cell, celln;
     bool listed;
 
+    __device__ __forceinline__ int entry(SkipLds<CELLS> &skl, const SkipArgs &sa, int kk, int &what) {
+        const int e = tile_at(skl, sa, listed, round, kk, nrun);
+        what = CELLS && listed ? enc_entry_cell(e) : 0;
+        return CELLS && listed ? enc_entry_tile(e) : e;
+    }
     template <int PS, bool TOKENS, class T, class Word>
-    __device__ __forceinline__ void begin(SkipLds &skl, const SkipArgs &sa, const TileSrc &src, int ntiles, int stagger,
+    __device__ __forceinline__ void begin(SkipLds<CELLS> &skl, const SkipArgs &sa, const TileSrc &src, int ntiles, int stagger,
                                           float *__restrict__ features, T *xs, Word word) {
         k = blockIdx.x;
-        nrun = tiles_to_run(skl, sa, ntiles);
-        listed = nrun != ntiles;
+        nrun = tiles_to_run(skl, sa, ntiles, listed);
         round = 0;
-        t = k < nrun ? tile_at(skl, sa, listed, 0, k, nrun) : 0;
-        if (listed && skip_fill_first()) skip_fill<PS, TOKENS>(sa, src.lg_tiles_x, features);
+        cell = 0;
+        t = k < nrun ? entry(skl, sa, k, cell) : 0;
+        if (listed && skip_fill_first()) skip_fill<PS, TOKENS, CELLS>(sa, src.lg_tiles_x, features);
         else if (stagger > 0 && ((blockIdx.x / 256) & 1))
             for (int i = 0; i < stagger; ++i) __builtin_amdgcn_s_sleep(127);
         const int tid = threadIdx.x;
         if (k < nrun) halo_to_lds(xs, src.fetch(t, tid), src.fetch(t, tid + 256), word);
         __syncthreads();
     }
-    __device__ __forceinline__ void next(SkipLds &skl, const SkipArgs &sa, const TileSrc &src, float &xr0, float &xr1) {
+    __device__ __forceinline__ void next(SkipLds<CELLS> &skl, const SkipArgs &sa, const TileSrc &src, float &xr0, float &xr1) {
         const int kn = k + gridDim.x;
         ++round;
-        tn = kn < nrun ? tile_at(skl, sa, listed, round, kn, nrun) : 0;
+        celln = 0;
+        tn = kn < nrun ? entry(skl, sa, kn, celln) : 0;
         xr0 = 0.f;
         xr1 = 0.f;
         if (kn < nrun) {
-            const int tid = threadIdx.x;
+            int tid = threadIdx.x;
+            if (CELLS) asm volatile("" : "+v"(tid));
             xr0 = src.fetch(tn, tid);
             xr1 = src.fetch(tn, tid + 256);
         }
@@ -602,8 +651,12 @@
     __device__ __forceinline__ void end(const SkipArgs &sa, const TileSrc &src, float *__restrict__ features) const {
         if (listed && !skip_fill_first()) {
             __builtin_amdgcn_s_setprio(0);
-            skip_fill<PS, TOKENS>(sa, src.lg_tiles_x, features);
-        }
+            skip_fill<PS, TOKENS, CELLS>(sa, src.lg_tiles_x, features);
+        }
+    }
+    __device__ __forceinline__ void advance() {
+        t = tn;
+        cell = celln;
     }
 };
 
@@ -764,8 +817,8 @@
     const int lane_off = (r >> 4) * 4 * B3_A1_ROW + (r & 15) * B3_A1_PITCH + 8 * hi * 2;
 
     const TileSrc src{frames, fstride, H, W, lg_tiles_x, lg_tiles_per_frame};
-    __shared__ SkipLds skl;
-    TileWalk wk;
+    __shared__ SkipLds<false> skl;
+    TileWalk<> wk;
     wk.begin<PS, TOKENS>(skl, sa, src, ntiles, stagger, features, xs, [](float v) { return v; });
 
     for (; wk.k < wk.nrun; wk.k += gridDim.x) {
@@ -871,7 +924,7 @@
 
         halo_to_lds(xs, xr0, xr1, [](float v) { return v; });
         __syncthreads();
-        wk.t = wk.tn;
+        wk.advance();
     }
     wk.end<PS, TOKENS>(sa, src, features);
 }
@@ -884,6 +937,7 @@
                                                      int lg_tiles_per_frame, int ntiles, int stagger,
                                                      SkipArgs sa) {
     extern __shared__ __attribute__((aligned(16))) unsigned char smem[];
+    constexpr bool CELLS = PS == 8;
     unsigned int *xs = reinterpret_cast<unsigned int *>(smem);
     unsigned char *a1h = smem + B3_XS_BYTES, *a1l = a1h + S16_A1_BYTES;
     unsigned char *w1s = a1l + S16_A1_BYTES;
@@ -919,13 +973,15 @@
         return (unsigned int)__builtin_bit_cast(unsigned short, vh) | ((unsigned int)__builtin_bit_cast(unsigned short, vl) << 16);
     };
     const TileSrc src{frames, fstride, H, W, lg_tiles_x, lg_tiles_per_frame};
-    __shared__ SkipLds skl;
-    TileWalk wk;
-    wk.begin<PS, TOKENS>(skl, sa, src, ntiles, stagger, features, xs, pack_split);
+    __shared__ SkipLds<CELLS> skl;
+    TileWalk<CELLS> wk;
+    wk.template begin<PS, TOKENS>(skl, sa, src, ntiles, stagger, features, xs, pack_split);
 
     for (; wk.k < wk.nrun; wk.k += gridDim.x) {
         int b, r0, c0;
         src.decode(wk.t, b, r0, c0);
+        int rt = r;
+        if (CELLS) asm volatile("" : "+v"(rt));
 
         __builtin_amdgcn_s_setprio(S16_PRIO_CONV1);
 #ifdef SMK_ENC_ABLATE
@@ -933,26 +989,31 @@
 #else
         constexpr bool abl_conv1 = true;
 #endif
+        auto x_build = [&](int ar, int ac, bf16x8 (&xh)[4], bf16x8 (&xl)[4]) {
+            const unsigned int *xp = xs + (ar + hi) * B3_XW + ac;
+            const unsigned int *xz = hi ? xs + (B3_XH - 1) * B3_XW + ac : xp + 6 * B3_XW;
+#pragma unroll
+            for (int s = 0; s < 4; ++s) {
+                unsigned int wh[4], wl[4];
+#pragma unroll
+                for (int jj = 0; jj < 4; ++jj) {
+                    const unsigned int *row = s == 3 ? xz : xp + s * 2 * B3_XW;
+                    const unsigned int e0 = row[2 * jj], e1 = jj == 3 ? 0u : row[2 * jj + 1];
+                    wh[jj] = __builtin_amdgcn_perm(e1, e0, 0x05040100u);
+                    wl[jj] = __builtin_amdgcn_perm(e1, e0, 0x07060302u);
+                }
+                xh[s] = __builtin_bit_cast(bf16x8, make_uint4(wh[0], wh[1], wh[2], wh[3]));
+                xl[s] = __builtin_bit_cast(bf16x8, make_uint4(wl[0], wl[1], wl[2], wl[3]));
+            }
+        };
         auto x_frags = [&](int pb, bf16x8 (&xh)[4], bf16x8 (&xl)[4], int &pix, bool &valid, bool &inimg) {
-            const int pp = pb * 32 + r;
+            const int pp = pb * 32 + rt;
             valid = pp < B3_APIX;
             pix = valid ? pp : B3_APIX - 1;
             const int ar = pix / B3_AW, ac = pix - ar * B3_AW;
             const int ii = r0 - 1 + ar, jj = c0 - 1 + ac;
             inimg = valid && ii >= 0 && ii < H && jj >= 0 && jj < W;
-            const unsigned int *xp = xs + (ar + hi) * B3_XW + ac;
-#pragma unroll
-            for (int s = 0; s < 4; ++s) {
-                unsigned int wh[4], wl[4];
-#pragma unroll
-                for (int jj = 0; jj < 4; ++jj) {
-                    const unsigned int e0 = xp[s * 2 * B3_XW + 2 * jj], e1 = xp[s * 2 * B3_XW + 2 * jj + 1];
-                    wh[jj] = __builtin_amdgcn_perm(e1, e0, 0x05040100u);
-                    wl[jj] = __builtin_amdgcn_perm(e1, e0, 0x07060302u);
-                }
-                xh[s] = __builtin_bit_cast(bf16x8, make_uint4(wh[0], wh[1], wh[2], wh[3]));
-                xl[s] = __builtin_bit_cast(bf16x8, make_uint4(wl[0], wl[1], wl[2], wl[3]));
-            }
+            x_build(ar, ac, xh, xl);
         };
         auto conv1_store = [&](const f32x16 &acc, int cb, int pix, bool valid, bool inimg) {
             const int sw = pix & 7;
@@ -977,162 +1038,286 @@
                 }
             }
         };
-        if (abl_conv1) {
-            bf16x8 xh[4], xl[4];
-            int pix; bool valid, inimg;
-            x_frags(wave, xh, xl, pix, valid, inimg);
-            f32x16 acc0, acc1;
-            conv1_both<true>(w1s, xh, xl, acc0, acc1);
-            conv1_store(acc0, 0, pix, valid, inimg);
-            conv1_store(acc1, 1, pix, valid, inimg);
-        }
-        if (abl_conv1) {
-            bf16x8 xh[4], xl[4];
-            int pix; bool valid, inimg;
-            const int cb = wave & 1;
-            x_frags(4 + (wave >> 1), xh, xl, pix, valid, inimg);
-            f32x16 acc;
-            conv1_one<true>(w1s, cb, xh, xl, acc);
-            conv1_store(acc, cb, pix, valid, inimg);
-        }
-#if !defined(SMK_ENC_ABLATE) || !(SMK_ENC_ABLATE & 4)
-        __syncthreads();
-#endif
-        __builtin_amdgcn_s_setprio(S16_PRIO_KLOOP);
-
-        float xr0, xr1;
-        wk.next(skl, sa, src, xr0, xr1);
-
-        f32x4v acc[8][2];
-#pragma unroll
-        for (int mt = 0; mt < 8; ++mt)
-#pragma unroll
-            for (int nt = 0; nt < 2; ++nt)
-#pragma unroll
-                for (int g = 0; g < 4; ++g) acc[mt][nt][g] = 0.f;
-        const int c16[2] = {kg << 4, (4 + kg) << 4};
-        auto tap_consts = [&](int ki, int kj, int (&om)[4]) {
-#pragma unroll
-            for (int m = 0; m < 4; ++m) om[m] = ((px + kj) << 7) ^ (((px + kj + 2 * (m + ki)) & 7) << 4);
-        };
-        auto load_a = [&](int ki, int half, int hm, const int (&om)[4], bf16x8 (&ah)[4], bf16x8 (&al)[4]) {
-            const unsigned char *ph = a1h + ki * (B3_AW * 128), *pl = a1l + ki * (B3_AW * 128);
-#pragma unroll
-            for (int m = 0; m < 4; ++m) {
-                const int off = om[m] ^ c16[half];
-                ah[m] = *reinterpret_cast<const bf16x8 *>(ph + off + (4 * hm + m) * (B3_AW * 128));
-                al[m] = *reinterpret_cast<const bf16x8 *>(pl + off + (4 * hm + m) * (B3_AW * 128));
-            }
-        };
-        bf16x8 ahA[4], alA[4], ahB[4], alB[4];
-        int om[4];
-        tap_consts(0, 0, om);
-        load_a(0, 0, 0, om, ahA, alA);
-        int ki = 0, kj = 0;
-#pragma unroll 1
-        for (int tap = 0; tap < 9; ++tap) {
-#pragma unroll
-            for (int u = 0; u < 4; ++u) {
-                const int half = u >> 1, hm = u & 1, slot = half % RING;
-                if (hm == 0) {
-                    int kn = tap * 2 + half + RING - 1;
-                    kn = kn >= 18 ? kn - 18 : kn;
-                    kn = __builtin_amdgcn_readfirstlane(kn);
-#pragma unroll
-                    for (int nt = 0; nt < 2; ++nt) {
-                        bq[(slot + RING - 1) % RING][nt][0] = load_b(kn, 0, nt);
-                        bq[(slot + RING - 1) % RING][nt][1] = load_b(kn, 1, nt);
-                    }
-                }
-                if (u < 3) {
-                    if (u & 1) load_a(ki, (u + 1) >> 1, (u + 1) & 1, om, ahA, alA);
-                    else load_a(ki, (u + 1) >> 1, (u + 1) & 1, om, ahB, alB);
-                } else if (tap < 8) {
-                    kj = kj == 2 ? 0 : kj + 1;
-                    ki = kj == 0 ? ki + 1 : ki;
-                    tap_consts(ki, kj, om);
-                    load_a(ki, 0, 0, om, ahA, alA);
-                }
-#pragma unroll
-                for (int pr = 0; pr < 3; ++pr)
-#pragma unroll
-                    for (int m = 0; m < 4; ++m)
-#pragma unroll
-                        for (int nt = 0; nt < 2; ++nt) {
-                            const bf16x8 bh = __builtin_bit_cast(bf16x8, bq[slot][nt][0]);
-                            const bf16x8 bl = __builtin_bit_cast(bf16x8, bq[slot][nt][1]);
-                            f32x4v &c = acc[4 * hm + m][nt];
-                            const bf16x8 ah = (u & 1) ? ahB[m] : ahA[m], al = (u & 1) ? alB[m] : alA[m];
-#if defined(SMK_ENC_ABLATE) && (SMK_ENC_ABLATE & 8)
-                            asm volatile("" :: "v"(al), "v"(ah), "v"(bh), "v"(bl), "v"(c));
-#else
-                            if (pr == 0) c = __builtin_amdgcn_mfma_f32_16x16x32_bf16(al, bh, c, 0, 0, 0);
-                            else if (pr == 1) c = __builtin_amdgcn_mfma_f32_16x16x32_bf16(ah, bl, c, 0, 0, 0);
-                            else c = __builtin_amdgcn_mfma_f32_16x16x32_bf16(ah, bh, c, 0, 0, 0);
-#endif
-                        }
-#pragma unroll
-                for (int i = 0; i < 24; ++i) {
-                    __builtin_amdgcn_sched_group_barrier(0x008, 1, 0);
-                    if (i % 3 == 0) __builtin_amdgcn_sched_group_barrier(0x100, 1, 0);
-                    else if (hm == 0 && (i == 1 || i == 2 || i == 4 || i == 5)) __builtin_amdgcn_sched_group_barrier(0x020, 1, 0);
-                }
-                __builtin_amdgcn_sched_barrier(0);
-            }
-        }
-
         auto out_index = [&](int pi, int pj, int o) -> size_t {
             return TOKENS ? ((size_t)b * 1024 + pi * 32 + pj) * 128 + o : ((size_t)b * 128 + o) * 1024 + pi * 32 + pj;
         };
+        float xr0, xr1;
+        if (CELLS && wk.cell != 0) {
+            const int side = wk.cell & 1;
+            int cpx = px, ckg = kg;
+            asm volatile("" : "+v"(cpx), "+v"(ckg));
+            uint4 bqx[2][2];
+            auto ring_load = [&](uint4 (&slot)[2][2], int ks) {
+#pragma unroll
+                for (int nt = 0; nt < 2; ++nt) {
+                    slot[nt][0] = load_b(ks, 0, nt);
+                    slot[nt][1] = load_b(ks, 1, nt);
+                }
+            };
+            ring_load(bq[1], 1);
+            if (abl_conv1) {
+                bf16x8 xh[4], xl[4];
+                const int pp = wave * 32 + rt;
+                const bool valid = pp < ENC_CELL_A1_PIX;
+                int ar, ac;
+                enc_cell_conv1_pixel(valid ? pp : ENC_CELL_A1_PIX - 1, side, ar, ac);
+                const int pix = ar * B3_AW + ac, ii = r0 - 1 + ar, jj = c0 - 1 + ac;
+                const bool inimg = valid && ii >= 0 && ii < H && jj >= 0 && jj < W;
+                x_build(ar, ac, xh, xl);
+                f32x16 acc0, acc1;
+                conv1_both<true>(w1s, xh, xl, acc0, acc1);
+                conv1_store(acc0, 0, pix, valid, inimg);
+                conv1_store(acc1, 1, pix, valid, inimg);
+            }
+            __syncthreads();
+            __builtin_amdgcn_s_setprio(S16_PRIO_KLOOP);
+            wk.next(skl, sa, src, xr0, xr1);
+
+            f32x4v acc[4][2];
+#pragma unroll
+            for (int m = 0; m < 4; ++m)
+#pragma unroll
+                for (int nt = 0; nt < 2; ++nt)
+#pragma unroll
+                    for (int g = 0; g < 4; ++g) acc[m][nt][g] = 0.f;
+            const int c16[2] = {ckg << 4, (4 + ckg) << 4};
+            const int pl = enc_cell_a1_pixel(0, cpx, 0, 0, side);
+            auto tap_consts = [&](int ki, int kj, int (&om)[2]) {
+#pragma unroll
+                for (int m = 0; m < 2; ++m) om[m] = ((pl + kj) << 7) ^ (((pl + kj + 2 * (2 * m + ki)) & 7) << 4);
+            };
+            auto load_a = [&](int ki, int half, const int (&om)[2], bf16x8 (&ah)[4], bf16x8 (&al)[4]) {
+                const unsigned char *ph = a1h + ki * (B3_AW * 128), *pw = a1l + ki * (B3_AW * 128);
+#pragma unroll
+                for (int m = 0; m < 4; ++m) {
+                    const int off = om[m & 1] ^ c16[half];
+                    ah[m] = *reinterpret_cast<const bf16x8 *>(ph + off + 2 * m * (B3_AW * 128));
+                    al[m] = *reinterpret_cast<const bf16x8 *>(pw + off + 2 * m * (B3_AW * 128));
+                }
+            };
+            bf16x8 ahA[4], alA[4], ahB[4], alB[4];
+            int om[2];
+            tap_consts(0, 0, om);
+            load_a(0, 0, om, ahA, alA);
+#pragma unroll 1
+            for (int ki = 0; ki < 3; ++ki) {
+#pragma unroll
+                for (int u = 0; u < 6; ++u) {
+                    const int kj = u >> 1, half = u & 1;
+                    uint4 (&bs)[2][2] = u % 3 == 0 ? bq[0] : u % 3 == 1 ? bq[1] : bqx;
+                    uint4 (&bn)[2][2] = (u + 2) % 3 == 0 ? bq[0] : (u + 2) % 3 == 1 ? bq[1] : bqx;
+                    if (u < 4) ring_load(bn, __builtin_amdgcn_readfirstlane(6 * ki + u + 2));
+                    else if (u == 4) ring_load(bn, __builtin_amdgcn_readfirstlane(ki < 2 ? 6 * ki + 6 : 0));
+                    else if (ki < 2) ring_load(bn, __builtin_amdgcn_readfirstlane(6 * ki + 7));
+                    if (u < 5) {
+                        if (u & 1) {
+                            tap_consts(ki, kj + 1, om);
+                            load_a(ki, 0, om, ahA, alA);
+                        } else {
+                            load_a(ki, 1, om, ahB, alB);
+                        }
+                    } else if (ki < 2) {
+                        tap_consts(ki + 1, 0, om);
+                        load_a(ki + 1, 0, om, ahA, alA);
+                    }
+#pragma unroll
+                    for (int pr = 0; pr < 3; ++pr)
+#pragma unroll
+                        for (int m = 0; m < 4; ++m)
+#pragma unroll
+                            for (int nt = 0; nt < 2; ++nt) {
+                                const bf16x8 bh = __builtin_bit_cast(bf16x8, bs[nt][0]);
+                                const bf16x8 bl = __builtin_bit_cast(bf16x8, bs[nt][1]);
+                                f32x4v &c = acc[m][nt];
+                                const bf16x8 ah = half ? ahB[m] : ahA[m], al = half ? alB[m] : alA[m];
+                                if (pr == 0) c = __builtin_amdgcn_mfma_f32_16x16x32_bf16(al, bh, c, 0, 0, 0);
+                                else if (pr == 1) c = __builtin_amdgcn_mfma_f32_16x16x32_bf16(ah, bl, c, 0, 0, 0);
+                                else c = __builtin_amdgcn_mfma_f32_16x16x32_bf16(ah, bh, c, 0, 0, 0);
+                            }
+#pragma unroll
+                    for (int i = 0; i < 24; ++i) {
+                        __builtin_amdgcn_sched_group_barrier(0x008, 1, 0);
+                        if (i % 3 == 0) __builtin_amdgcn_sched_group_barrier(0x100, 1, 0);
+                        else if (i == 1 || i == 2 || i == 4 || i == 5) __builtin_amdgcn_sched_group_barrier(0x020, 1, 0);
+                    }
+                    __builtin_amdgcn_sched_barrier(0);
+                }
+            }
+
+            float sum = 0.f;
+#pragma unroll
+            for (int m = 0; m < 4; ++m) {
+                float ev[4], od[4];
+#pragma unroll
+                for (int i = 0; i < 4; ++i) {
+                    const unsigned int va = __builtin_bit_cast(unsigned int, bn_relu(acc[m][0][i], s2a, t2a));
+                    const unsigned int vb = __builtin_bit_cast(unsigned int, bn_relu(acc[m][1][i], s2b, t2b));
+                    const auto sw = __builtin_amdgcn_permlane32_swap(va, vb, false, false);
+                    ev[i] = __builtin_bit_cast(float, (unsigned int)sw[0]);
+                    od[i] = __builtin_bit_cast(float, (unsigned int)sw[1]);
+                }
+#pragma unroll
+                for (int i = 0; i < 4; ++i) sum += ev[i];
+#pragma unroll
+                for (int i = 0; i < 4; ++i) sum += od[i];
+            }
+            const float other = __shfl_xor(sum, 16);
+            const float total = (ckg & 1) == 0 ? sum + other : other + sum;
+            if ((ckg & 1) == 0) features[out_index(r0 / 8, c0 / 8 + side, o0 + 16 * (ckg >> 1))] = total * (1.0f / 64);
+        } else {
+            if (abl_conv1) {
+                bf16x8 xh[4], xl[4];
+                int pix; bool valid, inimg;
+                x_frags(wave, xh, xl, pix, valid, inimg);
+                f32x16 acc0, acc1;
+                conv1_both<true>(w1s, xh, xl, acc0, acc1);
+                conv1_store(acc0, 0, pix, valid, inimg);
+                conv1_store(acc1, 1, pix, valid, inimg);
+            }
+            if (abl_conv1) {
+                bf16x8 xh[4], xl[4];
+                int pix; bool valid, inimg;
+                const int cb = wave & 1;
+                x_frags(4 + (wave >> 1), xh, xl, pix, valid, inimg);
+                f32x16 acc;
+                conv1_one<true>(w1s, cb, xh, xl, acc);
+                conv1_store(acc, cb, pix, valid, inimg);
+            }
+#if !defined(SMK_ENC_ABLATE) || !(SMK_ENC_ABLATE & 4)
+            __syncthreads();
+#endif
+            __builtin_amdgcn_s_setprio(S16_PRIO_KLOOP);
+
+            wk.next(skl, sa, src, xr0, xr1);
+
+            f32x4v acc[8][2];
+#pragma unroll
+            for (int mt = 0; mt < 8; ++mt)
+#pragma unroll
+                for (int nt = 0; nt < 2; ++nt)
+#pragma unroll
+                    for (int g = 0; g < 4; ++g) acc[mt][nt][g] = 0.f;
+            const int c16[2] = {kg << 4, (4 + kg) << 4};
+            auto tap_consts = [&](int ki, int kj, int (&om)[4]) {
+#pragma unroll
+                for (int m = 0; m < 4; ++m) om[m] = ((px + kj) << 7) ^ (((px + kj + 2 * (m + ki)) & 7) << 4);
+            };
+            auto load_a = [&](int ki, int half, int hm, const int (&om)[4], bf16x8 (&ah)[4], bf16x8 (&al)[4]) {
+                const unsigned char *ph = a1h + ki * (B3_AW * 128), *pl = a1l + ki * (B3_AW * 128);
+#pragma unroll
+                for (int m = 0; m < 4; ++m) {
+                    const int off = om[m] ^ c16[half];
+                    ah[m] = *reinterpret_cast<const bf16x8 *>(ph + off + (4 * hm + m) * (B3_AW * 128));
+                    al[m] = *reinterpret_cast<const bf16x8 *>(pl + off + (4 * hm + m) * (B3_AW * 128));
+                }
+            };
+            bf16x8 ahA[4], alA[4], ahB[4], alB[4];
+            int om[4];
+            tap_consts(0, 0, om);
+            load_a(0, 0, 0, om, ahA, alA);
+            int ki = 0, kj = 0;
+#pragma unroll 1
+            for (int tap = 0; tap < 9; ++tap) {
+#pragma unroll
+                for (int u = 0; u < 4; ++u) {
+                    const int half = u >> 1, hm = u & 1, slot = half % RING;
+                    if (hm == 0) {
+                        int kn = tap * 2 + half + RING - 1;
+                        kn = kn >= 18 ? kn - 18 : kn;
+                        kn = __builtin_amdgcn_readfirstlane(kn);
+#pragma unroll
+                        for (int nt = 0; nt < 2; ++nt) {
+                            bq[(slot + RING - 1) % RING][nt][0] = load_b(kn, 0, nt);
+                            bq[(slot + RING - 1) % RING][nt][1] = load_b(kn, 1, nt);
+                        }
+                    }
+                    if (u < 3) {
+                        if (u & 1) load_a(ki, (u + 1) >> 1, (u + 1) & 1, om, ahA, alA);
+                        else load_a(ki, (u + 1) >> 1, (u + 1) & 1, om, ahB, alB);
+                    } else if (tap < 8) {
+                        kj = kj == 2 ? 0 : kj + 1;
+                        ki = kj == 0 ? ki + 1 : ki;
+                        tap_consts(ki, kj, om);
+                        load_a(ki, 0, 0, om, ahA, alA);
+                    }
+#pragma unroll
+                    for (int pr = 0; pr < 3; ++pr)
+#pragma unroll
+                        for (int m = 0; m < 4; ++m)
+#pragma unroll
+                            for (int nt = 0; nt < 2; ++nt) {
+                                const bf16x8 bh = __builtin_bit_cast(bf16x8, bq[slot][nt][0]);
+                                const bf16x8 bl = __builtin_bit_cast(bf16x8, bq[slot][nt][1]);
+                                f32x4v &c = acc[4 * hm + m][nt];
+                                const bf16x8 ah = (u & 1) ? ahB[m] : ahA[m], al = (u & 1) ? alB[m] : alA[m];
+#if defined(SMK_ENC_ABLATE) && (SMK_ENC_ABLATE & 8)
+                                asm volatile("" :: "v"(al), "v"(ah), "v"(bh), "v"(bl), "v"(c));
+#else
+                                if (pr == 0) c = __builtin_amdgcn_mfma_f32_16x16x32_bf16(al, bh, c, 0, 0, 0);
+                                else if (pr == 1) c = __builtin_amdgcn_mfma_f32_16x16x32_bf16(ah, bl, c, 0, 0, 0);
+                                else c = __builtin_amdgcn_mfma_f32_16x16x32_bf16(ah, bh, c, 0, 0, 0);
+#endif
+                            }
+#pragma unroll
+                    for (int i = 0; i < 24; ++i) {
+                        __builtin_amdgcn_sched_group_barrier(0x008, 1, 0);
+                        if (i % 3 == 0) __builtin_amdgcn_sched_group_barrier(0x100, 1, 0);
+                        else if (hm == 0 && (i == 1 || i == 2 || i == 4 || i == 5)) __builtin_amdgcn_sched_group_barrier(0x020, 1, 0);
+                    }
+                    __builtin_amdgcn_sched_barrier(0);
+                }
+            }
+
 #if defined(SMK_ENC_ABLATE) && (SMK_ENC_ABLATE & 2)
 #pragma unroll
-        for (int mt = 0; mt < 8; ++mt) asm volatile("" :: "v"(acc[mt][0]), "v"(acc[mt][1]));
-        if (false)
+            for (int mt = 0; mt < 8; ++mt) asm volatile("" :: "v"(acc[mt][0]), "v"(acc[mt][1]));
+            if (false)
 #endif
 #pragma unroll
-        for (int nt = 0; nt < 2; ++nt) {
-            const float s2 = nt ? s2b : s2a, t2 = nt ? t2b : t2a;
-            const int o = o0 + 16 * nt;
-            if (PS == 2) {
-#pragma unroll
-                for (int mp = 0; mp < 4; ++mp)
-#pragma unroll
-                    for (int cg = 0; cg < 2; ++cg) {
+            for (int nt = 0; nt < 2; ++nt) {
+                const float s2 = nt ? s2b : s2a, t2 = nt ? t2b : t2a;
+                const int o = o0 + 16 * nt;
+                if (PS == 2) {
+#pragma unroll
+                    for (int mp = 0; mp < 4; ++mp)
+#pragma unroll
+                        for (int cg = 0; cg < 2; ++cg) {
+                            float sum = 0.f;
+#pragma unroll
+                            for (int mt = 2 * mp; mt < 2 * mp + 2; ++mt)
+#pragma unroll
+                                for (int i = 2 * cg; i < 2 * cg + 2; ++i) sum += bn_relu(acc[mt][nt][i], s2, t2);
+                            features[out_index((r0 + 2 * mp) / 2, (c0 + 4 * kg + 2 * cg) / 2, o)] = sum * 0.25f;
+                        }
+                } else if (PS == 4) {
+#pragma unroll
+                    for (int mq = 0; mq < 2; ++mq) {
                         float sum = 0.f;
 #pragma unroll
-                        for (int mt = 2 * mp; mt < 2 * mp + 2; ++mt)
-#pragma unroll
-                            for (int i = 2 * cg; i < 2 * cg + 2; ++i) sum += bn_relu(acc[mt][nt][i], s2, t2);
-                        features[out_index((r0 + 2 * mp) / 2, (c0 + 4 * kg + 2 * cg) / 2, o)] = sum * 0.25f;
+                        for (int mt = 4 * mq; mt < 4 * mq + 4; ++mt)
+#pragma unroll
+                            for (int i = 0; i < 4; ++i) sum += bn_relu(acc[mt][nt][i], s2, t2);
+                        features[out_index((r0 + 4 * mq) / 4, (c0 + 4 * kg) / 4, o)] = sum * (1.0f / 16);
                     }
-            } else if (PS == 4) {
-#pragma unroll
-                for (int mq = 0; mq < 2; ++mq) {
+                } else if (PS >= 16) {
                     float sum = 0.f;
 #pragma unroll
-                    for (int mt = 4 * mq; mt < 4 * mq + 4; ++mt)
+                    for (int mt = 0; mt < 8; ++mt)
 #pragma unroll
                         for (int i = 0; i < 4; ++i) sum += bn_relu(acc[mt][nt][i], s2, t2);
-                    features[out_index((r0 + 4 * mq) / 4, (c0 + 4 * kg) / 4, o)] = sum * (1.0f / 16);
-                }
-            } else if (PS >= 16) {
-                float sum = 0.f;
-#pragma unroll
-                for (int mt = 0; mt < 8; ++mt)
-#pragma unroll
-                    for (int i = 0; i < 4; ++i) sum += bn_relu(acc[mt][nt][i], s2, t2);
-                const float half8 = sum + __shfl_xor(sum, 16);
-                const float total = half8 + __shfl_xor(half8, 32);
-                if (kg == 0) features[(size_t)wk.t * 128 + o] = total;
-            } else {
-                float sum = 0.f;
-#pragma unroll
-                for (int mt = 0; mt < 8; ++mt)
-#pragma unroll
-                    for (int i = 0; i < 4; ++i) sum += bn_relu(acc[mt][nt][i], s2, t2);
-                const float other = __shfl_xor(sum, 16);
-                const float total = (kg & 1) == 0 ? sum + other : other + sum;
-                if ((kg & 1) == 0) features[out_index(r0 / 8, c0 / 8 + (kg >> 1), o)] = total * (1.0f / 64);
+                    const float half8 = sum + __shfl_xor(sum, 16);
+                    const float total = half8 + __shfl_xor(half8, 32);
+                    if (kg == 0) features[(size_t)wk.t * 128 + o] = total;
+                } else {
+                    float sum = 0.f;
+#pragma unroll
+                    for (int mt = 0; mt < 8; ++mt)
+#pragma unroll
+                        for (int i = 0; i < 4; ++i) sum += bn_relu(acc[mt][nt][i], s2, t2);
+                    const float other = __shfl_xor(sum, 16);
+                    const float total = (kg & 1) == 0 ? sum + other : other + sum;
+                    if ((kg & 1) == 0) features[out_index(r0 / 8, c0 / 8 + (kg >> 1), o)] = total * (1.0f / 64);
+                }
             }
         }
 
@@ -1140,17 +1325,18 @@
 #if !defined(SMK_ENC_ABLATE) || !(SMK_ENC_ABLATE & 4)
         __syncthreads();
 #endif
-        wk.t = wk.tn;
-    }
-    wk.end<PS, TOKENS>(sa, src, features);
+        wk.advance();
+    }
+    wk.template end<PS, TOKENS>(sa, src, features);
 }
 
 struct EncoderKnobs {
     int stagger, wgs_per_cu, shape;
-    bool skip;
+    bool skip, cells;
     EncoderKnobs() {
         const char *sv = getenv("SMK_ENC_STAGGER"), *ov = getenv("SMK_ENC_WGS_PER_CU"), *sh = getenv("SMK_ENC_SHAPE");
-        const char *sk = getenv("SMK_ENC_SKIP");
+        const char *sk = getenv("SMK_ENC_SKIP"), *ce = getenv("SMK_ENC_CELLS");
+        cells = !(ce && atoi(ce) == 0);
         stagger = sv ? atoi(sv) : 1;
         wgs_per_cu = ov && atoi(ov) > 0 ? atoi(ov) : 0;
         shape = sh && atoi(sh) == 32 ? 32 : 16;
@@ -1164,7 +1350,8 @@
 
 template <bool VEC, int ROWS>
 __global__ __launch_bounds__(256) void k_encoder_tile_scan(const float *__restrict__ frames, int64_t fstride, int H, int W, int lg_tiles_x,
-                                                           int bands_per_frame, unsigned long long *__restrict__ masks) {
+                                                           int bands_per_frame, unsigned long long *__restrict__ masks,
+                                                           unsigned long long *__restrict__ cell_l, unsigned long long *__restrict__ cell_r) {
     constexpr int SCAN_ROWS = ROWS;
     constexpr int SCAN_BR = 2 * ROWS + 2;
     constexpr int SCAN_FW = 1024 / ROWS / 4 + 2;
@@ -1191,16 +1378,22 @@
     }
     __syncthreads();
     if (tid < 64) {
-        unsigned int any = 0;
+        unsigned int any[2] = {0, 0};
         if (tid < band_tiles) {
             const int tyl = tid >> lg_tiles_x, tx = tid & (tiles_x - 1);
 #pragma unroll
-            for (int br = 0; br < 4; ++br)
-#pragma unroll
-                for (int bc = 0; bc < 6; ++bc) any |= flag[2 * tyl + br][4 * tx + bc];
-        }
-        const unsigned long long m = __ballot(any != 0);
-        if (tid == 0) masks[band] = m;
+            for (int side = 0; side < 2; ++side)
+#pragma unroll
+                for (int br = 0; br < 4; ++br)
+#pragma unroll
+                    for (int bc = 0; bc < ENC_CELL_FLAG_COLS; ++bc) any[side] |= flag[2 * tyl + br][enc_cell_flag_col(tx, side) + bc];
+        }
+        const unsigned long long l = __ballot(any[0] != 0), r = __ballot(any[1] != 0);
+        if (tid == 0) {
+            masks[band] = enc_cells_tile(l, r);
+            cell_l[band] = l;
+            cell_r[band] = r;
+        }
     }
 }
 
@@ -1267,16 +1460,19 @@
     if (sk->ws_bands < (size_t)nbands) {
         if (capturing) return hipSuccess;
         int *p = nullptr;
-        if ((err = hipMalloc((void **)&p, (4 + 2 * (size_t)nbands) * sizeof(int))) != hipSuccess) return err;
+        if ((err = hipMalloc((void **)&p, (4 + 6 * (size_t)nbands) * sizeof(int))) != hipSuccess) return err;
         if (sk->ws) sk->retired.push_back(sk->ws);
         sk->ws = p;
         sk->ws_bands = nbands;
     }
     int *count = sk->ws;
     unsigned long long *masks = reinterpret_cast<unsigned long long *>(sk->ws + 4);
+    unsigned long long *cell_l = masks + nbands, *cell_r = cell_l + nbands;
     const bool vec = (reinterpret_cast<uintptr_t>(frames) & 15) == 0 && (fstride & 3) == 0;
     dim3 grid(nbands), block(256);
-    auto scan = [&](auto kern) { hipLaunchKernelGGL(kern, grid, block, 0, st, frames, fstride, H, W, lg_tx, bands_per_frame, masks); };
+    auto scan = [&](auto kern) {
+        hipLaunchKernelGGL(kern, grid, block, 0, st, frames, fstride, H, W, lg_tx, bands_per_frame, masks, cell_l, cell_r);
+    };
     switch (scan_rows) {
         case 4: vec ? scan(k_encoder_tile_scan<true, 4>) : scan(k_encoder_tile_scan<false, 4>); break;
         case 2: vec ? scan(k_encoder_tile_scan<true, 2>) : scan(k_encoder_tile_scan<false, 2>); break;
@@ -1284,6 +1480,8 @@
     }
     if ((err = hipGetLastError()) != hipSuccess) return err;
     plan.masks = masks;
+    plan.cell_l = enc_knobs().cells ? cell_l : masks;
+    plan.cell_r = enc_knobs().cells ? cell_r : masks;
     plan.count = count;
     plan.nbands = nbands;
     plan.lg_band_tiles = lg_tx + 2 < 6 ? lg_tx + 2 : 6;
@@ -1338,8 +1536,8 @@
     const int lane_off = (r >> 4) * 4 * I8_A1_ROW + (r & 15) * I8_A1_PITCH + 16 * hi;
 
     const TileSrc src{frames, fstride, H, W, lg_tiles_x, lg_tiles_per_frame};
-    __shared__ SkipLds skl;
-    TileWalk wk;
+    __shared__ SkipLds<false> skl;
+    TileWalk<> wk;
     wk.begin<PS, TOKENS>(skl, sa, src, ntiles, 0, features, xs, [](float v) { return v; });
 
     for (; wk.k < wk.nrun; wk.k += gridDim.x) {
@@ -1492,7 +1690,7 @@
 
         halo_to_lds(xs, xr0, xr1, [](float v) { return v; });
         __syncthreads();
-        wk.t = wk.tn;
+        wk.advance();
     }
     wk.end<PS, TOKENS>(sa, src, features);
 }
diff --git a/smokephysai_amd/csrc/encoder_cells.h b/smokephysai_amd/csrc/encoder_cells.h
--- /dev/null
+++ b/smokephysai_amd/csrc/encoder_cells.h
@@ -0,0 +1,41 @@
+#pragma once
+#if defined(__HIPCC__) || defined(__CUDACC__)
+#define SMK_ENC_HD __host__ __device__ inline __attribute__((always_inline))
+#else
+#define SMK_ENC_HD inline
+#endif
+namespace smk {
+
+constexpr int ENC_CELL = 8;
+constexpr int ENC_CELL_HALO = 4;
+constexpr int ENC_CELL_A1 = ENC_CELL + 2;
+constexpr int ENC_CELL_A1_PIX = ENC_CELL_A1 * ENC_CELL_A1;
+constexpr int ENC_CELL_AW = 18;
+
+SMK_ENC_HD void enc_cell_window(int r0, int c0, int side, int &row_lo, int &row_hi, int &col_lo, int &col_hi) {
+    row_lo = r0 - ENC_CELL_HALO;
+    row_hi = r0 + ENC_CELL + ENC_CELL_HALO;
+    col_lo = c0 + ENC_CELL * side - ENC_CELL_HALO;
+    col_hi = c0 + ENC_CELL * side + ENC_CELL + ENC_CELL_HALO;
+}
+constexpr int ENC_CELL_FLAG_COLS = 4;
+SMK_ENC_HD int enc_cell_flag_col(int tx, int side) { return 4 * tx + 2 * side; }
+
+SMK_ENC_HD unsigned long long enc_cells_tile(unsigned long long l, unsigned long long r) { return l | r; }
+SMK_ENC_HD unsigned long long enc_cells_both(unsigned long long l, unsigned long long r) { return l & r; }
+SMK_ENC_HD unsigned long long enc_cells_one(unsigned long long l, unsigned long long r) { return l ^ r; }
+
+constexpr int ENC_ENTRY_SHIFT = 29, ENC_ENTRY_TILE = (1 << ENC_ENTRY_SHIFT) - 1;
+SMK_ENC_HD int enc_entry(int tile, bool one_cell, int side) { return tile | (one_cell ? (2 | side) << ENC_ENTRY_SHIFT : 0); }
+SMK_ENC_HD int enc_entry_tile(int entry) { return entry & ENC_ENTRY_TILE; }
+SMK_ENC_HD int enc_entry_cell(int entry) { return entry >> ENC_ENTRY_SHIFT; }
+
+SMK_ENC_HD void enc_cell_conv1_pixel(int pp, int side, int &ar, int &ac) {
+    ar = pp / ENC_CELL_A1;
+    ac = ENC_CELL * side + pp - ar * ENC_CELL_A1;
+}
+SMK_ENC_HD int enc_cell_a1_pixel(int m, int px, int ki, int kj, int side) {
+    return (2 * m + (px >> 3) + ki) * ENC_CELL_AW + ENC_CELL * side + (px & 7) + kj;
+}
+
+}
```

After: 242,900, median of 6. +2.3%, better.
